# nverchev/PointCloudCounterfactual

Hardware: AMD Instinct MI355X
Metric: clouds/sec Chamfer+EMD fwd+bwd, N=2048 B=32 (higher is better)
Workload: dtype f32; 1 GPU; BASELINE configs[1]+[2]: N=2048 B=32 per GPU, nn_distance (Chamfer, mean) fwd+bwd + match_cost (approxmatch+matchcost) fwd+bwd through the autograd surface; inputs = "recon" clouds (reference permuted + N(0, 0.02^2): a trained autoencoder, SURVEY 8(d)); the 8(d) stress set (both clouds i.i.d. U[0,1]^3) is value_stress (--full); emd_mode=implicit, batch_per_gpu=32, n_points=2048, global_batch=32, parallelism=batch-sharded x1, no data-path collective, launcher=single process

## Files before the change

### pointcloudcounterfactual_amd/backend.py

```python

from __future__ import annotations

import torch

from pointcloudcounterfactual_amd import _lib
from pointcloudcounterfactual_amd._lib import call, ptr

_L = _lib.lib
F32, I32 = torch.float32, torch.int32


def _sizes(set_d: torch.Tensor, set_q: torch.Tensor) -> tuple[int, int, int]:
    return set_d.size(0), set_d.size(1), set_q.size(1)


def ApproxMatch(set_d: torch.Tensor, set_q: torch.Tensor) -> list[torch.Tensor]:
    b, n, m = _sizes(set_d, set_q)
    dev = set_d.device
    match = torch.empty((b, m, n), dtype=torch.float32, device=dev)
    temp = torch.empty((b, (n + m) * 2), dtype=torch.float32, device=dev)
    call(_L.pcc_approxmatch, 'ApproxMatch', dev, b, n, m, ptr(set_d, 'set_d', F32, dev), ptr(set_q, 'set_q', F32, dev),
         ptr(match, 'match', F32, dev), ptr(temp, 'temp', F32, dev))
    return [match, temp]


def ApproxMatchCost(set_d: torch.Tensor, set_q: torch.Tensor) -> list[torch.Tensor]:
    b, n, m = _sizes(set_d, set_q)
    dev = set_d.device
    match = torch.empty((b, m, n), dtype=torch.float32, device=dev)
    temp = torch.empty((b, (n + m) * 2), dtype=torch.float32, device=dev)
    cost = torch.empty((b,), dtype=torch.float32, device=dev)
    call(_L.pcc_approxmatch_cost, 'ApproxMatchCost', dev, b, n, m, ptr(set_d, 'set_d', F32, dev),
         ptr(set_q, 'set_q', F32, dev), ptr(match, 'match', F32, dev), ptr(temp, 'temp', F32, dev),
         ptr(cost, 'cost', F32, dev))
    return [match, temp, cost]


def MatchCostImplicit(set_d: torch.Tensor, set_q: torch.Tensor, with_grad: bool) -> list[torch.Tensor]:
    b, n, m = _sizes(set_d, set_q)
    dev = set_d.device
    cost = torch.empty((b,), dtype=torch.float32, device=dev)
    out = [cost]
    g1 = g2 = None
    if with_grad:
        g1 = torch.empty((b, n, 3), dtype=torch.float32, device=dev)
        g2 = torch.empty((b, m, 3), dtype=torch.float32, device=dev)
        out += [g1, g2]
    call(_L.pcc_match_cost, 'MatchCostImplicit', dev, b, n, m, ptr(set_d, 'set_d', F32, dev),
         ptr(set_q, 'set_q', F32, dev), None, ptr(cost, 'cost', F32, dev), ptr(g1, 'grad1', F32, dev),
         ptr(g2, 'grad2', F32, dev))
    return out


def MatchCost(set_d: torch.Tensor, set_q: torch.Tensor, match: torch.Tensor) -> torch.Tensor:
    b, n, m = _sizes(set_d, set_q)
    dev = set_d.device
    out = torch.empty((b,), dtype=torch.float32, device=dev)
    if match.numel() != b * n * m:
        raise RuntimeError(f'match has {match.numel()} elements, expected {b}x{m}x{n}')
    call(_L.pcc_matchcost, 'MatchCost', dev, b, n, m, ptr(set_d, 'set_d', F32, dev), ptr(set_q, 'set_q', F32, dev),
         ptr(match, 'match', F32, dev), ptr(out, 'cost', F32, dev))
    return out


def MatchCostGrad(set_d: torch.Tensor, set_q: torch.Tensor, match: torch.Tensor) -> list[torch.Tensor]:
    b, n, m = _sizes(set_d, set_q)
    dev = set_d.device
    grad1 = torch.empty((b, n, 3), dtype=torch.float32, device=dev)
    grad2 = torch.empty((b, m, 3), dtype=torch.float32, device=dev)
    if match.numel() != b * n * m:
        raise RuntimeError(f'match has {match.numel()} elements, expected {b}x{m}x{n}')
    call(_L.pcc_matchcostgrad, 'MatchCostGrad', dev, b, n, m, ptr(set_d, 'set_d', F32, dev),
         ptr(set_q, 'set_q', F32, dev), ptr(match, 'match', F32, dev), ptr(grad1, 'grad1', F32, dev),
         ptr(grad2, 'grad2', F32, dev))
    return [grad1, grad2]


def MatchCostGradScaled(set_d: torch.Tensor, set_q: torch.Tensor, match: torch.Tensor,
                        grad_cost: torch.Tensor) -> list[torch.Tensor]:
    b, n, m = _sizes(set_d, set_q)
    dev = set_d.device
    grad1 = torch.empty((b, n, 3), dtype=torch.float32, device=dev)
    grad2 = torch.empty((b, m, 3), dtype=torch.float32, device=dev)
    if match.numel() != b * n * m or grad_cost.numel() != b:
        raise RuntimeError('MatchCostGradScaled: match / grad_cost shapes do not match the clouds')
    call(_L.pcc_matchcostgrad_scaled, 'MatchCostGradScaled', dev, b, n, m, ptr(set_d, 'set_d', F32, dev),
         ptr(set_q, 'set_q', F32, dev), ptr(match, 'match', F32, dev), ptr(grad_cost, 'grad_cost', F32, dev),
         ptr(grad1, 'grad1', F32, dev), ptr(grad2, 'grad2', F32, dev))
    return [grad1, grad2]


def NNDistance(set_d: torch.Tensor, set_q: torch.Tensor) -> list[torch.Tensor]:
    b, n, m = _sizes(set_d, set_q)
    dev = set_d.device
    dist1 = torch.empty((b, n), dtype=torch.float32, device=dev)
    idx1 = torch.empty((b, n), dtype=torch.int32, device=dev)
    dist2 = torch.empty((b, m), dtype=torch.float32, device=dev)
    idx2 = torch.empty((b, m), dtype=torch.int32, device=dev)
    call(_L.pcc_nndistance, 'NNDistance', dev, b, n, ptr(set_d, 'set_d', F32, dev), m, ptr(set_q, 'set_q', F32, dev),
         ptr(dist1, 'dist1', F32, dev), ptr(idx1, 'idx1', I32, dev), ptr(dist2, 'dist2', F32, dev),
         ptr(idx2, 'idx2', I32, dev))
    return [dist1, idx1, dist2, idx2]


def ChamferLoss(set_d: torch.Tensor, set_q: torch.Tensor, mean: bool) -> list[torch.Tensor]:
    b, n, m = _sizes(set_d, set_q)
    dev = set_d.device
    loss = torch.empty((b,), dtype=torch.float32, device=dev)
    dist1 = torch.empty((b, n), dtype=torch.float32, device=dev)
    idx1 = torch.empty((b, n), dtype=torch.int32, device=dev)
    dist2 = torch.empty((b, m), dtype=torch.float32, device=dev)
    idx2 = torch.empty((b, m), dtype=torch.int32, device=dev)
    call(_L.pcc_chamfer_loss, 'ChamferLoss', dev, b, n, ptr(set_d, 'set_d', F32, dev), m, ptr(set_q, 'set_q', F32, dev),
         int(mean), ptr(loss, 'loss', F32, dev), ptr(dist1, 'dist1', F32, dev), ptr(idx1, 'idx1', I32, dev),
         ptr(dist2, 'dist2', F32, dev), ptr(idx2, 'idx2', I32, dev))
    return [loss, dist1, idx1, dist2, idx2]


def ChamferLossGrad(set_d: torch.Tensor, set_q: torch.Tensor, idx1: torch.Tensor, idx2: torch.Tensor,
                    grad_loss: torch.Tensor, mean: bool) -> list[torch.Tensor]:
    b, n, m = _sizes(set_d, set_q)
    dev = set_d.device
    grad1 = torch.empty((b, n, 3), dtype=torch.float32, device=dev)
    grad2 = torch.empty((b, m, 3), dtype=torch.float32, device=dev)
    if idx1.numel() != b * n or idx2.numel() != b * m or grad_loss.numel() != b:
        raise RuntimeError('ChamferLossGrad: idx / grad_loss shapes do not match the clouds')
    grad_loss, stride = _batch_stride(grad_loss, b)
    call(_L.pcc_chamfer_loss_grad, 'ChamferLossGrad', dev, b, n, ptr(set_d, 'set_d', F32, dev), m,
         ptr(set_q, 'set_q', F32, dev), ptr(idx1, 'idx1', I32, dev), ptr(idx2, 'idx2', I32, dev),
         ptr(grad_loss, 'grad_loss', F32, dev), stride, int(mean), ptr(grad1, 'grad1', F32, dev),
         ptr(grad2, 'grad2', F32, dev))
    return [grad1, grad2]


def ChamferEMD(set_d: torch.Tensor, set_q: torch.Tensor, mean: bool, with_grad: bool,
               return_dist: bool = False) -> list[torch.Tensor]:
    b, n, m = _sizes(set_d, set_q)
    dev = set_d.device
    loss = torch.empty((b,), dtype=torch.float32, device=dev)
    idx1 = torch.empty((b, n), dtype=torch.int32, device=dev)
    idx2 = torch.empty((b, m), dtype=torch.int32, device=dev)
    cost = torch.empty((b,), dtype=torch.float32, device=dev)
    out = [loss, idx1, idx2, cost]
    g1 = g2 = None
    if with_grad:
        g1 = torch.empty((b, n, 3), dtype=torch.float32, device=dev)
        g2 = torch.empty((b, m, 3), dtype=torch.float32, device=dev)
        out += [g1, g2]
    d1 = torch.empty((b, n), dtype=torch.float32, device=dev)
    d2 = torch.empty((b, m), dtype=torch.float32, device=dev)
    call(_L.pcc_chamfer_emd, 'ChamferEMD', dev, b, n, ptr(set_d, 'set_d', F32, dev), m, ptr(set_q, 'set_q', F32, dev),
         int(mean), ptr(loss, 'loss', F32, dev), ptr(d1, 'dist1', F32, dev), ptr(idx1, 'idx1', I32, dev),
         ptr(d2, 'dist2', F32, dev), ptr(idx2, 'idx2', I32, dev), ptr(cost, 'cost', F32, dev),
         ptr(g1, 'emd_grad1', F32, dev), ptr(g2, 'emd_grad2', F32, dev))
    if return_dist:
        out += [d1, d2]
    return out


def _batch_stride(g: torch.Tensor, b: int) -> tuple[torch.Tensor, int]:
    stride = g.stride(0) if g.dim() == 1 and b > 1 else 1
    if stride == 0:
        return g[:1], 0
    if stride != 1:
        return g.contiguous(), 1
    return g, 1


def ChamferEMDGrad(set_d: torch.Tensor, set_q: torch.Tensor, idx1: torch.Tensor, idx2: torch.Tensor,
                   grad_chamfer: torch.Tensor, mean: bool, emd_grad1: torch.Tensor, emd_grad2: torch.Tensor,
                   grad_emd: torch.Tensor) -> list[torch.Tensor]:
    b, n, m = _sizes(set_d, set_q)
    dev = set_d.device
    grad1 = torch.empty((b, n, 3), dtype=torch.float32, device=dev)
    grad2 = torch.empty((b, m, 3), dtype=torch.float32, device=dev)
    if (idx1.numel() != b * n or idx2.numel() != b * m or grad_chamfer.numel() != b or grad_emd.numel() != b
            or emd_grad1.numel() != b * n * 3 or emd_grad2.numel() != b * m * 3):
        raise RuntimeError('ChamferEMDGrad: shapes do not match the clouds')
    grad_chamfer, sc = _batch_stride(grad_chamfer, b)
    grad_emd, se = _batch_stride(grad_emd, b)
    call(_L.pcc_chamfer_emd_grad, 'ChamferEMDGrad', dev, b, n, ptr(set_d, 'set_d', F32, dev), m,
         ptr(set_q, 'set_q', F32, dev), ptr(idx1, 'idx1', I32, dev), ptr(idx2, 'idx2', I32, dev),
         ptr(grad_chamfer, 'grad_chamfer', F32, dev), sc, int(mean), ptr(emd_grad1, 'emd_grad1', F32, dev),
         ptr(emd_grad2, 'emd_grad2', F32, dev), ptr(grad_emd, 'grad_emd', F32, dev), se, ptr(grad1, 'grad1', F32, dev),
         ptr(grad2, 'grad2', F32, dev))
    return [grad1, grad2]


def NNDistanceGrad(set_d: torch.Tensor, set_q: torch.Tensor, idx1: torch.Tensor, idx2: torch.Tensor,
                   grad_dist1: torch.Tensor, grad_dist2: torch.Tensor) -> list[torch.Tensor]:
    b, n, m = _sizes(set_d, set_q)
    dev = set_d.device
    grad1 = torch.empty((b, n, 3), dtype=torch.float32, device=dev)
    grad2 = torch.empty((b, m, 3), dtype=torch.float32, device=dev)
    if idx1.numel() != b * n or grad_dist1.numel() != b * n or idx2.numel() != b * m or grad_dist2.numel() != b * m:
        raise RuntimeError('NNDistanceGrad: idx/grad_dist shapes do not match the clouds')
    call(_L.pcc_nndistancegrad, 'NNDistanceGrad', dev, b, n, ptr(set_d, 'set_d', F32, dev), m,
         ptr(set_q, 'set_q', F32, dev), ptr(grad_dist1, 'grad_dist1', F32, dev), ptr(idx1, 'idx1', I32, dev),
         ptr(grad_dist2, 'grad_dist2', F32, dev), ptr(idx2, 'idx2', I32, dev), ptr(grad1, 'grad1', F32, dev),
         ptr(grad2, 'grad2', F32, dev))
    return [grad1, grad2]
```

### pointcloudcounterfactual_amd/csrc/am_pair.hip

```cpp
#include "approxmatch.hpp"
#include "wave_ops.hpp"

#include <algorithm>

namespace {

using pcc::sq3;

constexpr int kPairRB = 8;
constexpr int kPairPad = 65;

struct PairArgs {
    int n, m, n4, m4;
    const float *soa1, *soa2;
    const float *lv;
    LevelConsts lc;
    float cut2[kLevels];
    float *cost_part;
    float *part1;
    float *part2;
    int col_blocks, row_tiles, bc;
};

template <int Q, bool GRAD>
__global__ __launch_bounds__(256) void am_pair_kernel(PairArgs a) {
    __shared__ float4 lds_l[kPairRT][3];
    __shared__ int lds_mask[kPairRT];
    __shared__ float stash[GRAD ? 4 * kPairRB * 3 * kPairPad : 4];
    __shared__ float lds_red[4];
    const int tid = threadIdx.x, lane = tid & 63;
    const int w = __builtin_amdgcn_readfirstlane(tid >> 6);
    const int cbn = a.col_blocks, rtn = a.row_tiles;
    const int item = (int)blockIdx.x / a.bc, smp = (int)blockIdx.x - item * a.bc;
    const int shift_k = item / cbn, cblk = item - shift_k * cbn;
    const int base_r = (int)(((long long)(2 * cblk + 1) * rtn) / (2 * cbn));
    const int shift = ((shift_k + 1) >> 1) * ((shift_k & 1) ? 1 : -1);
    const int rtile = ((base_r + shift) % rtn + rtn) % rtn;
    const int l0 = rtile * kPairRT;
    const int kb = cblk * 64 * Q;
    const int k0 = kb + lane * Q;
    const size_t nm4 = (size_t)a.n4 + a.m4;
    const float *lvb = a.lv + (size_t)smp * kLevels * nm4;
    const float *s1 = a.soa1 + (size_t)smp * 3 * a.n4;
    const float *s2 = a.soa2 + (size_t)smp * 3 * a.m4;
    const int lcnt = min(kPairRT, a.m - l0);

    float rowx = 0.f, rowy = 0.f, rowz = 0.f, rowr[kLevels];
#pragma unroll
    for (int i = 0; i < kLevels; i++) rowr[i] = 0.f;
    if (tid < lcnt) {
        const int l = l0 + tid;
        rowx = s2[l];
        rowy = s2[a.m4 + l];
        rowz = s2[2 * a.m4 + l];
#pragma unroll
        for (int i = 0; i < kLevels; i++) rowr[i] = lvb[(size_t)i * nm4 + a.n4 + l];
    }
    float x1[Q], y1[Q], z1[Q], rl[kLevels][Q];
    float blo[3] = {__builtin_inff(), __builtin_inff(), __builtin_inff()};
    float bhi[3] = {-__builtin_inff(), -__builtin_inff(), -__builtin_inff()};
#pragma unroll
    for (int q = 0; q < Q; q++) {
        const bool real = k0 + q < a.n;
        const int k = real ? k0 + q : a.n - 1;
        x1[q] = s1[k];
        y1[q] = s1[a.n4 + k];
        z1[q] = s1[2 * a.n4 + k];
#pragma unroll
        for (int i = 0; i < kLevels; i++) rl[i][q] = real ? lvb[(size_t)i * nm4 + k] : 0.f;
        blo[0] = fminf(blo[0], x1[q]); bhi[0] = fmaxf(bhi[0], x1[q]);
        blo[1] = fminf(blo[1], y1[q]); bhi[1] = fmaxf(bhi[1], y1[q]);
        blo[2] = fminf(blo[2], z1[q]); bhi[2] = fmaxf(bhi[2], z1[q]);
    }
#pragma unroll
    for (int c = 0; c < 3; c++) {
#pragma unroll
        for (int off = 1; off < 64; off <<= 1) {
            blo[c] = fminf(blo[c], __shfl_xor(blo[c], off, 64));
            bhi[c] = fmaxf(bhi[c], __shfl_xor(bhi[c], off, 64));
        }
    }
    if (tid < lcnt) {
        const float bx = fmaxf(fmaxf(blo[0] - rowx, rowx - bhi[0]), 0.f);
        const float by = fmaxf(fmaxf(blo[1] - rowy, rowy - bhi[1]), 0.f);
        const float bz = fmaxf(fmaxf(blo[2] - rowz, rowz - bhi[2]), 0.f);
        const float bd2 = bx * bx + by * by + bz * bz;
        int mask = 0;
#pragma unroll
        for (int i = 0; i < kLevels; i++) mask |= (rowr[i] != 0.f && !(bd2 > a.cut2[i])) ? (1 << i) : 0;
        lds_l[tid][0] = make_float4(rowx, rowy, rowz, rowr[0]);
        lds_l[tid][1] = make_float4(rowr[1], rowr[2], rowr[3], rowr[4]);
        lds_l[tid][2] = make_float4(rowr[5], rowr[6], rowr[7], rowr[8]);
        lds_mask[tid] = mask;
    }
    float g1[Q][3];
#pragma unroll
    for (int q = 0; q < Q; q++) g1[q][0] = g1[q][1] = g1[q][2] = 0.f;
    float csum = 0.f;
    float *my_stash = stash + (GRAD ? w * kPairRB * 3 * kPairPad : 0);
    __syncthreads();

    for (int base = 0; base < lcnt; base += 4 * kPairRB) {
#pragma unroll 1
        for (int s = 0; s < kPairRB; s++) {
            const int li = base + 4 * s + w;
            float rx = 0.f, ry = 0.f, rz = 0.f;
            const int mask = li < lcnt ? __builtin_amdgcn_readfirstlane(lds_mask[li]) : 0;
            if (mask) {
                const float4 A = lds_l[li][0], B = lds_l[li][1], Cc = lds_l[li][2];
                const float rr[kLevels] = {A.w, B.x, B.y, B.z, B.w, Cc.x, Cc.y, Cc.z, Cc.w};
                float ex[Q], ey[Q], ez[Q], d[Q], acc[Q];
#pragma unroll
                for (int q = 0; q < Q; q++) {
                    ex[q] = A.x - x1[q];
                    ey[q] = A.y - y1[q];
                    ez[q] = A.z - z1[q];
                    d[q] = sq3(ex[q], ey[q], ez[q]);
                    acc[q] = 0.f;
                }
#pragma unroll
                for (int i = 0; i < kLevels; i++) {
                    if (mask & (1 << i)) {
#pragma unroll
                        for (int q = 0; q < Q; q++)
                            acc[q] = __builtin_fmaf(fast_exp2(a.lc.c[i] * d[q]) * rl[i][q], rr[i], acc[q]);
                    }
                }
#pragma unroll
                for (int q = 0; q < Q; q++) {
                    if (GRAD) {
                        float dm;
                        asm("v_max_f32 %0, %1, %2" : "=v"(dm) : "v"(d[q]), "v"(1e-20f));
                        const float f = acc[q] * __builtin_amdgcn_rsqf(dm);
                        csum = __builtin_fmaf(f, d[q], csum);
                        g1[q][0] = __builtin_fmaf(-ex[q], f, g1[q][0]);
                        g1[q][1] = __builtin_fmaf(-ey[q], f, g1[q][1]);
                        g1[q][2] = __builtin_fmaf(-ez[q], f, g1[q][2]);
                        rx = __builtin_fmaf(ex[q], f, rx);
                        ry = __builtin_fmaf(ey[q], f, ry);
                        rz = __builtin_fmaf(ez[q], f, rz);
                    } else {
                        csum = __builtin_fmaf(acc[q], __builtin_amdgcn_sqrtf(d[q]), csum);
                    }
                }
            }
            if (GRAD) {
                my_stash[(s * 3 + 0) * kPairPad + lane] = rx;
                my_stash[(s * 3 + 1) * kPairPad + lane] = ry;
                my_stash[(s * 3 + 2) * kPairPad + lane] = rz;
            }
        }
        if (GRAD) {
            const int v = lane % 24, h = lane / 24;
            float t = 0.f;
            __builtin_amdgcn_wave_barrier();
            if (lane < 48) {
                const float *src = my_stash + v * kPairPad + h * 32;
#pragma unroll 8
                for (int i = 0; i < 32; i++) t += src[i];
            }
            __builtin_amdgcn_wave_barrier();
            const float hi = __shfl(t, lane + 24, 64);
            const int sl = v / 3, c = v - sl * 3;
            const int li = base + 4 * sl + w;
            if (lane < 24 && li < lcnt)
                a.part2[(((size_t)smp * cbn + cblk) * a.m4 + (l0 + li)) * 3 + c] = t + hi;
        }
    }
    csum = pcc::wave_sum_down(csum);
    if (lane == 0) lds_red[w] = csum;
    __syncthreads();
    if (tid == 0)
        a.cost_part[(size_t)smp * cbn * rtn + rtile * cbn + cblk] =
            ((lds_red[0] + lds_red[1]) + lds_red[2]) + lds_red[3];
    if (GRAD) {
        static_assert(Q * 3 * 64 <= 4 * kPairRB * 3 * kPairPad, "column merge reuses the stash");
        for (int src = 1; src < 4; src++) {
            __syncthreads();
            if (w == src) {
#pragma unroll
                for (int q = 0; q < Q; q++)
#pragma unroll
                    for (int c = 0; c < 3; c++) stash[(q * 3 + c) * 64 + lane] = g1[q][c];
            }
            __syncthreads();
            if (w == 0) {
#pragma unroll
                for (int q = 0; q < Q; q++)
#pragma unroll
                    for (int c = 0; c < 3; c++) g1[q][c] += stash[(q * 3 + c) * 64 + lane];
            }
        }
        if (w == 0) {
            float *dst = a.part1 + (((size_t)smp * rtn + rtile) * a.n4) * 3;
#pragma unroll
            for (int q = 0; q < Q; q++) {
                if (k0 + q < a.n) {
#pragma unroll
                    for (int c = 0; c < 3; c++) dst[(size_t)(k0 + q) * 3 + c] = g1[q][c];
                }
            }
        }
    }
}

struct FinishArgs {
    int parts[3], npts[2], pitch[2];
    const float *part[3];
    const int *perm[2];
    const float *scale;
    float *out[3];
    const float *ch_d1, *ch_d2;
    float *ch_loss;
    int ch_n, ch_m, ch_mean;
    const int *flags;
};
__global__ __launch_bounds__(256) void pair_finish_kernel(FinishArgs f) {
    __shared__ float red[256];
    const int which = blockIdx.z, smp = blockIdx.y, tid = threadIdx.x;
    if (which == 3) {
        if (blockIdx.x) return;
        __shared__ float red2[256];
        float s1 = 0.f, s2 = 0.f;
        auto strided_sum = [&](const float *d, int cnt) -> float {
            float acc = 0.f;
            for (int i0 = tid; i0 < cnt; i0 += 8 * 256) {
                float v[8];
#pragma unroll
                for (int u = 0; u < 8; u++) v[u] = d[min(i0 + u * 256, cnt - 1)];
#pragma unroll
                for (int u = 0; u < 8; u++)
                    if (i0 + u * 256 < cnt) acc += v[u];
            }
            return acc;
        };
        s1 = strided_sum(f.ch_d1 + (size_t)smp * f.ch_n, f.ch_n);
        s2 = strided_sum(f.ch_d2 + (size_t)smp * f.ch_m, f.ch_m);
        red[tid] = s1;
        red2[tid] = s2;
        __syncthreads();
        for (int off = 128; off > 0; off >>= 1) {
            if (tid < off) {
                red[tid] += red[tid + off];
                red2[tid] += red2[tid + off];
            }
            __syncthreads();
        }
        if (tid == 0) f.ch_loss[smp] = f.ch_mean ? red2[0] / (float)f.ch_m + red[0] / (float)f.ch_n : red[0] + red2[0];
        return;
    }
    const bool poisoned = f.flags && (f.flags[(size_t)smp * kLiveRow + kInfSlot] | f.flags[(size_t)smp * kLiveRow + kInfSlot + 1] |
                                      f.flags[(size_t)smp * kLiveRow + kErrSlot]);
    if (which == 2) {
        if (blockIdx.x) return;
        const int parts = f.parts[2];
        float s = 0.f;
        for (int i = tid; i < parts; i += 256) s += f.part[2][(size_t)smp * parts + i];
        red[tid] = s;
        __syncthreads();
        for (int off = 128; off > 0; off >>= 1) {
            if (tid < off) red[tid] += red[tid + off];
            __syncthreads();
        }
        if (tid == 0) f.out[2][smp] = poisoned ? __builtin_nanf("") : red[0];
        return;
    }
    if (!f.out[which]) return;
    const int npts = f.npts[which], pitch = f.pitch[which], parts = f.parts[which];
    const int i = blockIdx.x * 256 + tid;
    if (i >= npts * 3) return;
    const int s = i / 3, c = i - s * 3;
    const float *p = f.part[which] + (size_t)smp * parts * pitch * 3 + i;
    const int pt = f.perm[which][(size_t)smp * npts + s];
    const size_t stride = (size_t)pitch * 3;
    float acc = p[0];
    int t = 1;
    for (; t + 8 <= parts; t += 8) {
        float v[8];
#pragma unroll
        for (int u = 0; u < 8; u++) v[u] = p[(size_t)(t + u) * stride];
#pragma unroll
        for (int u = 0; u < 8; u++) acc += v[u];
    }
    {
        float v[7];
#pragma unroll
        for (int u = 0; u < 7; u++) v[u] = p[(size_t)min(t + u, parts - 1) * stride];
#pragma unroll
        for (int u = 0; u < 7; u++)
            if (t + u < parts) acc += v[u];
    }
    f.out[which][((size_t)smp * npts + pt) * 3 + c] = poisoned ? __builtin_nanf("") : f.scale ? acc * f.scale[smp] : acc;
}

template <int Q>
int launch_pair(const PairArgs &pa, dim3 grid, bool grad, hipStream_t st) {
    pcc::ProfScope prof(grad ? "am_pair_kernel<grad>" : "am_pair_kernel<cost>", st);
    if (grad) hipLaunchKernelGGL((am_pair_kernel<Q, true>), grid, dim3(256), 0, st, pa);
    else hipLaunchKernelGGL((am_pair_kernel<Q, false>), grid, dim3(256), 0, st, pa);
    return pcc::check_launch("match_cost(pair)");
}

}

namespace pcc {

int launch_pair_finish(const AmDims &L, const WsView &v, int s0, int bc, int col_blocks, int row_tiles, const float *grad_cost,
                       float *cost, float *grad1, float *grad2, const ChamferOut *chamfer, hipStream_t lst) {
    const size_t o = (size_t)s0;
    const int n = L.n, m = L.m;
    const bool grad = grad1 && grad2;
    const LevelConsts lc = make_levels();
    PairArgs pa{};
    pa.n = n; pa.m = m; pa.n4 = L.n4; pa.m4 = L.m4;
    pa.soa1 = v.soa1; pa.soa2 = v.soa2; pa.lv = v.lv;
    pa.lc = lc;
    for (int i = 0; i < kLevels; i++) pa.cut2[i] = zero_cut2(lc, i);
    pa.cost_part = v.pair_cost;
    pa.part1 = grad ? v.part1 : nullptr;
    pa.part2 = grad ? v.part2 : nullptr;
    pa.col_blocks = col_blocks; pa.row_tiles = row_tiles; pa.bc = bc;
    if ((long long)col_blocks * row_tiles * bc > 0x7fffffffLL) return pcc::invalid("match_cost: grid too large");
    const dim3 grid((unsigned)(col_blocks * row_tiles * bc));
    if (int rc = launch_pair<kPairQ>(pa, grid, grad, lst)) return rc;
    FinishArgs f{};
    f.parts[0] = row_tiles; f.parts[1] = col_blocks; f.parts[2] = col_blocks * row_tiles;
    f.npts[0] = n; f.npts[1] = m; f.pitch[0] = L.n4; f.pitch[1] = L.m4;
    f.part[0] = pa.part1; f.part[1] = pa.part2; f.part[2] = pa.cost_part;
    f.perm[0] = v.perm1; f.perm[1] = v.perm2;
    f.scale = grad_cost ? grad_cost + o : nullptr;
    f.out[0] = grad ? grad1 + o * n * 3 : nullptr;
    f.out[1] = grad ? grad2 + o * m * 3 : nullptr;
    f.out[2] = cost + o;
    f.flags = v.live_cnt;
    if (chamfer) {
        f.ch_d1 = chamfer->dist1 + o * n; f.ch_d2 = chamfer->dist2 + o * m; f.ch_loss = chamfer->loss + o;
        f.ch_n = n; f.ch_m = m; f.ch_mean = chamfer->mean;
    }
    {
        pcc::ProfScope prof("pair_finish_kernel", lst);
        const int blocks = grad ? pcc::ceil_div(std::max(n, m) * 3, 256) : 1;
        hipLaunchKernelGGL(pair_finish_kernel, dim3(blocks, bc, chamfer ? 4 : 3), dim3(256), 0, lst, f);
    }
    return pcc::check_launch("match_cost(reduce)");
}
}
```

### pointcloudcounterfactual_amd/csrc/approxmatch.hip

```cpp
#include "approxmatch.hpp"
#include "pcc_test_hooks.h"
#include "wave_ops.hpp"

#include <algorithm>
#include <functional>
#include <mutex>
#include <type_traits>

namespace {

using pcc::sq3;
using pcc::WsView;

enum Phase { PH_A = 0, PH_B = 1, PH_CA = 2, PH_C = 3 };

__device__ __forceinline__ float pass_a_ratio(float remL, float sum) { return remL / (1e-9f + sum); }
struct PassB {
    float ratio, remain;
};
__device__ __forceinline__ PassB pass_b(float remR, float sum) {
    const float sumr = sum * remR;
    const float consumption = __builtin_fminf(remR / (sumr + 1e-9f), 1.0f);
    return {consumption * remR, __builtin_fmaxf(0.0f, remR - sumr)};
}
__device__ __forceinline__ float pass_c_left(float remL, float ratioL, float sum) { return __builtin_fmaxf(0.0f, remL - ratioL * sum); }

struct PhaseArgs {
    int n_own, n_cand, tiles, batch;
    int own_n4, cand_n4, own_nb, cand_nb;
    const float *own_soa, *cand_soa;
    const float *cand_box;
    const float *own_box16;
    const float *w0, *w1;
    long long w0_stride, w1_stride;
    float w0c;
    float c0, c1;
    float cut2;
    float cut2_fine;
    int first;
    int level;
    float multiL, multiR;
    float *remain;
    float *remain_out;
    long long remain_stride;
    const float *ratio_in;
    float *ratio_out;
    long long ratio_stride;
    float *clist;
    int *clist_cnt;
    int cl_n4;
    const unsigned *mask_in;
    unsigned *mask_out;
    int mask_words;
    const int *live_in;
    int *live_out;
};

enum Var { V_PLAIN = 0, V_CULL = 1, V_COWN = 3, V_CLIST = 4 };

struct Sched {
    int n, m, n4, m4, nb1, nb2;
    const float *soa1, *soa2, *box1, *box2;
    float *rem, *lv;
    float multiL, multiR;
    float *clist;
    int *clist_cnt;
    int *live_cnt;
    unsigned *live_mask;
    int skip;
    LevelConsts lc;
};

inline int sched_phases() { return 2 * kLevels + 1; }

inline PhaseArgs build_phase(const Sched &sc, int p, int *mode_out, int *var_out) {
    const long long nm4 = (long long)sc.n4 + sc.m4;
    const long long rs = (long long)sc.n4 + 2LL * sc.m4;
    PhaseArgs a{};
    a.multiL = sc.multiL;
    a.multiR = sc.multiR;
    const bool set1_owns = (p == 0) || (p % 2 == 0);
    if (set1_owns) {
        a.n_own = sc.n; a.n_cand = sc.m; a.own_n4 = sc.n4; a.cand_n4 = sc.m4; a.own_nb = sc.nb1; a.cand_nb = sc.nb2;
        a.own_soa = sc.soa1; a.cand_soa = sc.soa2; a.cand_box = sc.box2;
        a.own_box16 = sc.box1;
    } else {
        a.n_own = sc.m; a.n_cand = sc.n; a.own_n4 = sc.m4; a.cand_n4 = sc.n4; a.own_nb = sc.nb2; a.cand_nb = sc.nb1;
        a.own_soa = sc.soa2; a.cand_soa = sc.soa1; a.cand_box = sc.box1;
        a.own_box16 = sc.box2;
    }
    int mode, var;
    if (p == 0) {
        mode = PH_A;
        var = sc.skip ? V_CULL : V_PLAIN;
        a.level = 0;
        a.w0 = nullptr; a.w0c = sc.multiR; a.c0 = sc.lc.c[0]; a.first = 1;
        a.cut2 = zero_cut2(sc.lc, 0);
        a.ratio_out = sc.lv; a.ratio_stride = kLevels * nm4;
    } else {
        const int i = (p - 1) / 2;
        float *ratioL = sc.lv + (size_t)i * nm4, *ratioR = ratioL + sc.n4;
        a.level = i;
        a.first = (i == 0);
        a.c0 = sc.lc.c[i];
        if (p % 2 == 1) {
            mode = PH_B;
            var = !sc.skip ? V_PLAIN : i <= 2 ? V_CULL : V_COWN;
            a.w0 = ratioL; a.w0_stride = kLevels * nm4;
            a.cut2 = zero_cut2(sc.lc, i);
            a.remain = sc.rem + sc.n4 + (i & 1) * sc.m4;
            a.remain_out = sc.rem + sc.n4 + ((i + 1) & 1) * sc.m4;
            a.remain_stride = rs;
            a.ratio_out = ratioR; a.ratio_stride = kLevels * nm4;
            if (var == V_COWN) { a.clist = sc.clist; a.clist_cnt = sc.clist_cnt; a.cl_n4 = sc.m4; }
            if (sc.live_mask) {
                const int words = mask_words(sc.m4);
                a.mask_words = words;
                if (i + 1 < kLevels && (var == V_COWN || i == 2)) a.mask_out = sc.live_mask + (size_t)(i + 1) * words;
                if (var == V_COWN) {
                    a.mask_in = sc.live_mask + (size_t)i * words;
                    a.remain = a.remain_out = sc.rem + sc.n4 + sc.m4;
                }
            }
            if (sc.live_cnt) {
                a.live_in = (var == V_COWN && i >= 1) ? sc.live_cnt + i : nullptr;
                a.live_out = i + 1 < kLevels ? sc.live_cnt + i + 1 : nullptr;
            }
        } else {
            mode = i + 1 < kLevels ? PH_CA : PH_C;
            var = !sc.skip ? V_PLAIN : i <= 2 ? V_CULL : V_CLIST;
            if (var == V_CLIST) { a.clist = sc.clist; a.clist_cnt = sc.clist_cnt; a.cl_n4 = sc.m4; }
            a.w0 = ratioR; a.w0_stride = kLevels * nm4;
            a.w1 = sc.rem + sc.n4 + ((i + 1) & 1) * sc.m4; a.w1_stride = rs;
            a.remain = sc.rem; a.remain_stride = rs;
            a.ratio_in = ratioL; a.ratio_stride = kLevels * nm4;
            const int lc_i = i + 1 < kLevels ? i + 1 : i;
            a.cut2 = zero_cut2(sc.lc, lc_i);
            a.cut2_fine = zero_cut2(sc.lc, i);
            if (i + 1 < kLevels) {
                a.c1 = sc.lc.c[i + 1];
                a.ratio_out = sc.lv + (size_t)(i + 1) * nm4;
            }
        }
    }
    *mode_out = mode;
    *var_out = var;
    return a;
}

template <int NW, int R, int S, int CH>
struct PhaseLds {
    static constexpr int kC = (3 + NW) * CH;
    static constexpr int kRed = NW * S * 64 * R;
    static constexpr int kOwn = 64 * R;
    static constexpr int kWave = S;
    static constexpr int floats = kC + kRed + kOwn + kWave + 4;
};

template <int MODE, int R, int S, int CH, int VAR, int G = 1>
__device__ __forceinline__ void am_phase_body(const PhaseArgs &a, int smp, int tile, float *smem) {
    constexpr int T = 64 * S;
    constexpr int TQ = 64 * R / G;
    constexpr int PQ = 64 * R;
    static_assert(G == 1 || (VAR == V_COWN && R == 1), "lane-split owners: owner-compacted launches only");
    constexpr int NW = (MODE == PH_CA) ? 2 : 1;
    constexpr bool W0_CONST = (MODE == PH_A);
    constexpr bool COWN = VAR == V_COWN, CLIST = VAR == V_CLIST;
    static_assert(VAR == V_PLAIN || COWN || CLIST, "the box-culled passes run on am_fine_kernel");
    static_assert(!(CLIST && W0_CONST), "pass A of the first level has constant weights");
    static_assert(TQ <= T, "one epilogue owner per thread");
    using L = PhaseLds<NW, R, S, CH>;
    float *lds_c = smem;
    float *red = smem + L::kC;
    int *own_idx = reinterpret_cast<int *>(red + L::kRed);
    int *wave_cnt = own_idx + L::kOwn;

    const int tid = threadIdx.x;
    const int lane = tid & 63;
    const int w = __builtin_amdgcn_readfirstlane(tid >> 6);
    const int sub = G > 1 ? lane / TQ : 0;
    const float *O = a.own_soa + (size_t)smp * 3 * a.own_n4;
    const float *C = a.cand_soa + (size_t)smp * 3 * a.cand_n4;
    const float *W0 = W0_CONST ? nullptr : a.w0 + (size_t)smp * a.w0_stride;
    const float *W1 = (NW == 2) ? a.w1 + (size_t)smp * a.w1_stride : nullptr;

    if (!COWN && tile * TQ >= a.n_own) return;
    static_assert(CH / 4 <= T, "one float4 group per thread and chunk");
    float4 st_x, st_y, st_z, st_0, st_1;
    auto stage_load = [&](const float *Cc, const float *W0c, const float *W1c, int pitch, int q0, int ngroups) {
        const int i = min(tid, max(ngroups - 1, 0));
        st_x = reinterpret_cast<const float4 *>(Cc + q0)[i];
        st_y = reinterpret_cast<const float4 *>(Cc + (size_t)pitch + q0)[i];
        st_z = reinterpret_cast<const float4 *>(Cc + (size_t)2 * pitch + q0)[i];
        st_0 = make_float4(a.w0c, a.w0c, a.w0c, a.w0c);
        st_1 = st_0;
        if (!W0_CONST) st_0 = *reinterpret_cast<const float4 *>(W0c + q0 + 4 * i);
        if (NW == 2) st_1 = *reinterpret_cast<const float4 *>(W1c + q0 + 4 * i);
    };
    if (COWN) stage_load(C, W0, W1, a.cand_n4, 0, (min(CH, a.n_cand) + 3) / 4);
    int n_valid = min(TQ, a.n_own - tile * TQ);
    if (COWN) {
        const int lo = tile * TQ, hi = lo + TQ;
        const unsigned *mk = a.mask_in + (size_t)smp * kLevels * a.mask_words;
        unsigned *mnext = (tile == 0 && a.mask_out) ? a.mask_out + (size_t)smp * kLevels * a.mask_words : nullptr;
        const int wpt = (a.mask_words + T - 1) / T;
        unsigned word = 0;
        int mine = 0;
        if (wpt == 1) {
            word = mk[min(tid, a.mask_words - 1)];
            word &= -(unsigned)(tid < a.mask_words);
            if (mnext && tid < a.mask_words) atomicAnd(&mnext[tid], word);
            mine = __popc(word);
        } else {
            for (int j = tid * wpt; j < min(tid * wpt + wpt, a.mask_words); j++) {
                const unsigned wj = mk[j];
                if (mnext) atomicAnd(&mnext[j], wj);
                mine += __popc(wj);
            }
        }
        int incl = mine;
#pragma unroll
        for (int off = 1; off < 64; off <<= 1) {
            const int v = __shfl_up(incl, off, 64);
            incl += lane >= off ? v : 0;
        }
        if (lane == 63) wave_cnt[w] = incl;
        __syncthreads();
        int before = 0, total = 0;
#pragma unroll
        for (int i = 0; i < S; i++) {
            const int c = __builtin_amdgcn_readfirstlane(wave_cnt[i]);
            before += i < w ? c : 0;
            total += c;
        }
        int pos = before + incl - mine - lo;
        auto deal = [&](unsigned bits, int first_owner) {
            while (bits) {
                const int bit = __builtin_ctz(bits);
                bits &= bits - 1;
                if ((unsigned)pos < (unsigned)TQ) own_idx[pos] = first_owner + bit;
                pos++;
            }
        };
        if (wpt == 1) {
            deal(word, tid * 32);
        } else {
            for (int j = tid * wpt; j < min(tid * wpt + wpt, a.mask_words); j++) deal(mk[j], j * 32);
        }
        if (a.clist_cnt && tile == 0 && tid == 0) a.clist_cnt[smp] = total;
        n_valid = min(TQ, total - lo);
        if (n_valid <= 0) return;
        (void)hi;
        __syncthreads();
    }
    int own_e = -1;
    if (tid < TQ && tid < n_valid) own_e = COWN ? own_idx[tid] : tile * TQ + tid;

    float ox[R], oy[R], oz[R], s0[R], s1[R];
    float t0x = 0.f, t1x = 0.f;
#pragma unroll
    for (int r = 0; r < R; r++) {
        const int e = G > 1 ? (lane & (TQ - 1)) : r * 64 + lane;
        int o = COWN ? own_idx[e < n_valid ? e : 0] : tile * TQ + e;
        o = o < a.n_own ? o : a.n_own - 1;
        ox[r] = O[o];
        oy[r] = O[a.own_n4 + o];
        oz[r] = O[2 * a.own_n4 + o];
        s0[r] = 0.f;
        s1[r] = 0.f;
    }
    float pre_rem = 0.f, pre_ratio = 0.f;
    {
        const int oe = max(own_e, 0);
        if (MODE != PH_A && !a.first) pre_rem = a.remain[(size_t)smp * a.remain_stride + oe];
        if (MODE == PH_CA || MODE == PH_C) pre_ratio = a.ratio_in[(size_t)smp * a.ratio_stride + oe];
    }
    const float4 *X4 = reinterpret_cast<const float4 *>(lds_c);
    const float4 *Y4 = X4 + CH / 4;
    const float4 *Z4 = Y4 + CH / 4;
    const float4 *A4 = Z4 + CH / 4;
    const float4 *B4 = A4 + CH / 4;
    const float c0 = a.c0, c1 = a.c1;

    const int n_cand = CLIST ? __builtin_amdgcn_readfirstlane(a.clist_cnt[smp]) : a.n_cand;
    if (CLIST) {
        C = a.clist + (size_t)smp * 5 * a.cl_n4;
        W0 = C + (size_t)3 * a.cl_n4;
        W1 = C + (size_t)4 * a.cl_n4;
    }
    const int cand_pitch = CLIST ? a.cl_n4 : a.cand_n4;
    for (int q0 = 0; q0 < n_cand; q0 += CH) {
        const int cnt = min(CH, n_cand - q0);
        int ngroups = (cnt + 3) / 4;
        if (q0) __syncthreads();
        {
            float4 *dst4 = reinterpret_cast<float4 *>(lds_c);
            if (!(COWN && q0 == 0)) stage_load(C, W0, W1, cand_pitch, q0, ngroups);
            const int i = tid;
            if (i < ngroups) {
                float4 vx = st_x, vy = st_y, vz = st_z, v0 = st_0, v1 = st_1;
                if (CLIST && i * 4 + 3 >= cnt) {
                    vx.y = i * 4 + 1 < cnt ? vx.y : 0.f; vx.z = i * 4 + 2 < cnt ? vx.z : 0.f; vx.w = 0.f;
                    vy.y = i * 4 + 1 < cnt ? vy.y : 0.f; vy.z = i * 4 + 2 < cnt ? vy.z : 0.f; vy.w = 0.f;
                    vz.y = i * 4 + 1 < cnt ? vz.y : 0.f; vz.z = i * 4 + 2 < cnt ? vz.z : 0.f; vz.w = 0.f;
                }
                if ((W0_CONST || CLIST) && i * 4 + 3 >= cnt) {
                    v0.x = i * 4 + 0 < cnt ? v0.x : 0.f;
                    v0.y = i * 4 + 1 < cnt ? v0.y : 0.f;
                    v0.z = i * 4 + 2 < cnt ? v0.z : 0.f;
                    v0.w = 0.f;
                    if (NW == 2) {
                        v1.x = i * 4 + 0 < cnt ? v1.x : 0.f;
                        v1.y = i * 4 + 1 < cnt ? v1.y : 0.f;
                        v1.z = i * 4 + 2 < cnt ? v1.z : 0.f;
                        v1.w = 0.f;
                    }
                }
                dst4[i] = vx;
                dst4[CH / 4 + i] = vy;
                dst4[2 * (CH / 4) + i] = vz;
                dst4[3 * (CH / 4) + i] = v0;
                if (NW == 2) dst4[4 * (CH / 4) + i] = v1;
            }
        }
        const int nblk = (ngroups + 3) / 4;
        __syncthreads();
        for (int blk = w; blk < nblk; blk += S) {
            const int g_end = min(blk * 4 + 4, ngroups);
            for (int g = blk * 4 + sub; g < g_end; g += G) {
                const float4 x = X4[g], y = Y4[g], z = Z4[g], wa = A4[g];
                float4 wb;
                if (NW == 2) wb = B4[g];
#pragma unroll
                for (int r = 0; r < R; r++) {
                    const float d0 = sq3(x.x - ox[r], y.x - oy[r], z.x - oz[r]);
                    const float d1 = sq3(x.y - ox[r], y.y - oy[r], z.y - oz[r]);
                    const float d2 = sq3(x.z - ox[r], y.z - oy[r], z.z - oz[r]);
                    const float d3 = sq3(x.w - ox[r], y.w - oy[r], z.w - oz[r]);
                    if (R == 1) {
                        s0[r] = __builtin_fmaf(fast_exp2(c0 * d0), wa.x, s0[r]);
                        t0x = __builtin_fmaf(fast_exp2(c0 * d1), wa.y, t0x);
                        s0[r] = __builtin_fmaf(fast_exp2(c0 * d2), wa.z, s0[r]);
                        t0x = __builtin_fmaf(fast_exp2(c0 * d3), wa.w, t0x);
                        if (NW == 2) {
                            s1[r] = __builtin_fmaf(fast_exp2(c1 * d0), wb.x, s1[r]);
                            t1x = __builtin_fmaf(fast_exp2(c1 * d1), wb.y, t1x);
                            s1[r] = __builtin_fmaf(fast_exp2(c1 * d2), wb.z, s1[r]);
                            t1x = __builtin_fmaf(fast_exp2(c1 * d3), wb.w, t1x);
                        }
                    } else {
                        s0[r] = __builtin_fmaf(fast_exp2(c0 * d0), wa.x, s0[r]);
                        s0[r] = __builtin_fmaf(fast_exp2(c0 * d1), wa.y, s0[r]);
                        s0[r] = __builtin_fmaf(fast_exp2(c0 * d2), wa.z, s0[r]);
                        s0[r] = __builtin_fmaf(fast_exp2(c0 * d3), wa.w, s0[r]);
                        if (NW == 2) {
                            s1[r] = __builtin_fmaf(fast_exp2(c1 * d0), wb.x, s1[r]);
                            s1[r] = __builtin_fmaf(fast_exp2(c1 * d1), wb.y, s1[r]);
                            s1[r] = __builtin_fmaf(fast_exp2(c1 * d2), wb.z, s1[r]);
                            s1[r] = __builtin_fmaf(fast_exp2(c1 * d3), wb.w, s1[r]);
                        }
                    }
                }
            }
        }
    }
    if (R == 1) {
        s0[0] += t0x;
        s1[0] += t1x;
    }
    if (G > 1) {
        s0[0] += __shfl_xor(s0[0], TQ, 64);
        if (G == 4) s0[0] += __shfl_xor(s0[0], 2 * TQ, 64);
    }
#pragma unroll
    for (int r = 0; r < R; r++) {
        red[(0 * S + w) * PQ + r * 64 + lane] = s0[r];
        if (NW == 2) red[(1 * S + w) * PQ + r * 64 + lane] = s1[r];
    }
    __syncthreads();
    if (own_e < 0) return;
    {
        const int e = tid;
        const int o = own_e;
        float t0 = red[e], t1 = 0.f;
        if (NW == 2) t1 = red[(1 * S) * PQ + e];
#pragma unroll
        for (int s = 1; s < S; s++) {
            t0 += red[(0 * S + s) * PQ + e];
            if (NW == 2) t1 += red[(1 * S + s) * PQ + e];
        }
        if (MODE == PH_A) {
            a.ratio_out[(size_t)smp * a.ratio_stride + o] = pass_a_ratio(a.multiL, t0);
        } else if (MODE == PH_B) {
            const PassB pb = pass_b(a.first ? a.multiR : pre_rem, t0);
            const float ratio_new = pb.ratio, remain_new = pb.remain;
            a.ratio_out[(size_t)smp * a.ratio_stride + o] = ratio_new;
            a.remain_out[(size_t)smp * a.remain_stride + o] = remain_new;
            if (a.live_out) {
                const unsigned long long alive = __ballot(remain_new != 0.f);
                if (lane == 0) atomicAdd(&a.live_out[(size_t)smp * kLiveRow], (int)__popcll(alive));
            }
            if (COWN && a.mask_out && remain_new == 0.f)
                atomicAnd(&a.mask_out[(size_t)smp * kLevels * a.mask_words + (o >> 5)], ~(1u << (o & 31)));
            if (COWN && a.clist) {
                float cx = ox[0], cy = oy[0], cz = oz[0];
#pragma unroll
                for (int r = 1; r < R; r++) {
                    cx = w == r ? ox[r] : cx;
                    cy = w == r ? oy[r] : cy;
                    cz = w == r ? oz[r] : cz;
                }
                float *cl = a.clist + (size_t)smp * 5 * a.cl_n4 + tile * TQ + e;
                cl[0] = cx;
                cl[(size_t)a.cl_n4] = cy;
                cl[(size_t)2 * a.cl_n4] = cz;
                cl[(size_t)3 * a.cl_n4] = ratio_new;
                cl[(size_t)4 * a.cl_n4] = remain_new;
            }
        } else {
            const float left = pass_c_left(a.first ? a.multiL : pre_rem, pre_ratio, t0);
            a.remain[(size_t)smp * a.remain_stride + o] = left;
            if (MODE == PH_CA) a.ratio_out[(size_t)smp * a.ratio_stride + o] = pass_a_ratio(left, t1);
        }
    }
}

template <int MODE, int R, int S, int CH, int VAR, int G = 1>
__global__ __launch_bounds__(64 * S) void am_phase_kernel(PhaseArgs a) {
    __shared__ __attribute__((aligned(16))) float smem[PhaseLds<(MODE == PH_CA ? 2 : 1), R, S, CH>::floats];
    constexpr bool COWN = VAR == V_COWN;
    int smp, tile;
    const int bid = (int)blockIdx.x, nwg = (int)gridDim.x;
    if (COWN) {
        if (a.batch % 8 == 0) {
            const int per = a.batch / 8, i = bid / 8;
            smp = (bid % 8) + 8 * (i % per);
            tile = i / per;
        } else {
            smp = bid % a.batch;
            tile = bid / a.batch;
        }
        if (a.live_in && tile > 0 && tile * (64 * R / G) >= a.live_in[(size_t)smp * kLiveRow]) return;
    } else {
        const int lid = pcc::xcd_contiguous(bid, nwg);
        smp = lid / a.tiles;
        tile = lid - smp * a.tiles;
    }
    am_phase_body<MODE, R, S, CH, VAR, G>(a, smp, tile, smem);
}

constexpr int kFineS = 8;
constexpr int kFineOG = 16;
constexpr int kFineGroups = 64 / kFineOG;
constexpr int kFineQ = 4;

struct FineOwners {
    float x[kFineQ], y[kFineQ], z[kFineQ];
};
struct FineRows {
    const float *x, *y, *z, *w0, *w1;
};

__device__ __forceinline__ void fine_group_box(const float *own_box, int own_nb, int smp, int g16, float4 &lo, float4 &hi) {
    lo = make_float4(__builtin_inff(), __builtin_inff(), __builtin_inff(), 0.f);
    hi = make_float4(-__builtin_inff(), -__builtin_inff(), -__builtin_inff(), 0.f);
    if (g16 < own_nb) {
        const float4 *ob = reinterpret_cast<const float4 *>(own_box + ((size_t)smp * own_nb + g16) * 8);
        lo = ob[0];
        hi = ob[1];
    }
}

__device__ __forceinline__ float fine_box_d2(const float4 &glo, const float4 &ghi, const float *cand_box) {
    const float4 *cb = reinterpret_cast<const float4 *>(cand_box);
    const float4 lo = cb[0], hi = cb[1];
    const float dx = fmaxf(fmaxf(glo.x - hi.x, lo.x - ghi.x), 0.f);
    const float dy = fmaxf(fmaxf(glo.y - hi.y, lo.y - ghi.y), 0.f);
    const float dz = fmaxf(fmaxf(glo.z - hi.z, lo.z - ghi.z), 0.f);
    return dx * dx + dy * dy + dz * dz;
}

template <int NBLK>
__device__ __forceinline__ void fine_block_list(bool keep, bool outer_only, int tid, int tg, int tb, int w, int lane,
                                                int *wave_cnt, unsigned char (*items)[NBLK], unsigned char *need) {
    if (tid < NBLK) need[tid] = 0;
    const unsigned long long bal = __ballot(keep);
    if (lane == 0) wave_cnt[w] = __popcll(bal);
    __syncthreads();
    const int before = (w & 1) ? wave_cnt[w - 1] : 0;
    if (keep) {
        items[tg][before + __popcll(bal & ((1ull << lane) - 1ull))] = (unsigned char)(tb | (outer_only ? 128 : 0));
        need[tb] = 1;
    }
    __syncthreads();
}

template <int NW>
__device__ __forceinline__ void fine_walk(const FineRows &rows, const unsigned char *list, int nitems, int cs, int cl, float c0,
                                          float c1, const FineOwners &own, float (&s0)[kFineQ], float (&s1)[kFineQ]) {
    for (int it = cs; it < nitems; it += 2) {
        const int item = __builtin_amdgcn_readfirstlane((int)list[it]);
        const int ci = (item & 127) * kBox + cl;
        const float x = rows.x[ci], y = rows.y[ci], z = rows.z[ci];
        if (NW == 2 && (item & 128)) {
            const float wb = rows.w1[ci];
#pragma unroll
            for (int j = 0; j < kFineQ; j++) s1[j] = __builtin_fmaf(fast_exp2(c1 * sq3(x - own.x[j], y - own.y[j], z - own.z[j])), wb, s1[j]);
            continue;
        }
        const float wa = rows.w0[ci];
        float wb = 0.f;
        if (NW == 2) wb = rows.w1[ci];
#pragma unroll
        for (int j = 0; j < kFineQ; j++) {
            const float d = sq3(x - own.x[j], y - own.y[j], z - own.z[j]);
            s0[j] = __builtin_fmaf(fast_exp2(c0 * d), wa, s0[j]);
            if (NW == 2) s1[j] = __builtin_fmaf(fast_exp2(c1 * d), wb, s1[j]);
        }
    }
}

template <int NW>
__device__ __forceinline__ void fine_reduce(float (&s0)[kFineQ], float (&s1)[kFineQ], float (*red)[2][64], int cs, int cl, int og, int quad) {
    const auto add = [](float a, float b) { return a + b; };
#pragma unroll
    for (int j = 0; j < kFineQ; j++) {
        s0[j] = pcc::row_reduce16(s0[j], add);
        if (NW == 2) s1[j] = pcc::row_reduce16(s1[j], add);
    }
    if (cl == 0) {
#pragma unroll
        for (int j = 0; j < kFineQ; j++) {
            red[0][cs][og * kFineOG + quad * kFineQ + j] = s0[j];
            if (NW == 2) red[1][cs][og * kFineOG + quad * kFineQ + j] = s1[j];
        }
    }
}

template <int MODE, int CH>
__global__ __launch_bounds__(64 * kFineS, MODE == PH_CA ? 4 : 8) void am_fine_kernel(PhaseArgs a) {
    constexpr int T = 64 * kFineS;
    constexpr int NW = (MODE == PH_CA) ? 2 : 1;
    constexpr bool W0_CONST = (MODE == PH_A);
    constexpr int NBLK = CH / kBox;
    static_assert(kFineGroups * NBLK == T, "one (owner group, candidate block) box test per thread");
    static_assert(kFineOG == kBox && kFineOG * kFineQ == 64, "a wave = 16 candidates x 4 owner quads");
    __shared__ __attribute__((aligned(16))) float lds_c[(3 + NW) * CH];
    __shared__ float red[NW][2][64];
    __shared__ unsigned char items[kFineGroups][NBLK];
    __shared__ unsigned char need[NBLK];
    __shared__ int wave_cnt[kFineS];

    const int lid = pcc::xcd_contiguous((int)blockIdx.x, (int)gridDim.x);
    const int smp = lid / a.tiles;
    const int tile = lid - smp * a.tiles;
    const int tid = threadIdx.x, lane = tid & 63;
    const int w = __builtin_amdgcn_readfirstlane(tid >> 6);
    const int og = w & (kFineGroups - 1);
    const int cs = w / kFineGroups;
    const int cl = lane & (kBox - 1);
    const int quad = lane / kBox;
    const float *O = a.own_soa + (size_t)smp * 3 * a.own_n4;
    const float *C = a.cand_soa + (size_t)smp * 3 * a.cand_n4;
    const float *W0 = W0_CONST ? nullptr : a.w0 + (size_t)smp * a.w0_stride;
    const float *W1 = (NW == 2) ? a.w1 + (size_t)smp * a.w1_stride : nullptr;

    FineOwners own;
    float s0[kFineQ], s1[kFineQ];
#pragma unroll
    for (int j = 0; j < kFineQ; j++) {
        int o = tile * 64 + og * kFineOG + quad * kFineQ + j;
        o = o < a.n_own ? o : a.n_own - 1;
        own.x[j] = O[o];
        own.y[j] = O[a.own_n4 + o];
        own.z[j] = O[2 * a.own_n4 + o];
        s0[j] = 0.f;
        s1[j] = 0.f;
    }
    const int own_e = (tid < 64 && tile * 64 + tid < a.n_own) ? tile * 64 + tid : -1;
    float pre_rem = 0.f, pre_ratio = 0.f;
    {
        const int oe = max(own_e, 0);
        if (MODE != PH_A && !a.first) pre_rem = a.remain[(size_t)smp * a.remain_stride + oe];
        if (MODE == PH_CA || MODE == PH_C) pre_ratio = a.ratio_in[(size_t)smp * a.ratio_stride + oe];
    }
    const int tg = tid / NBLK, tb = tid - tg * NBLK;
    float4 glo, ghi;
    fine_group_box(a.own_box16, a.own_nb, smp, tile * kFineGroups + tg, glo, ghi);
    const float c0 = a.c0, c1 = a.c1, cut2 = a.cut2;
    const FineRows rows = {lds_c, lds_c + CH, lds_c + 2 * CH, lds_c + 3 * CH, lds_c + 4 * CH};

    for (int q0 = 0; q0 < a.n_cand; q0 += CH) {
        const int cnt = min(CH, a.n_cand - q0);
        const int ngroups = (cnt + 3) / 4;
        const int nblk = (ngroups + 3) / 4;
        if (q0) __syncthreads();
        bool keep = false, outer_only = false;
        if (tb < nblk) {
            const float bd2 = fine_box_d2(glo, ghi, a.cand_box + ((size_t)smp * a.cand_nb + q0 / kBox + tb) * 8);
            keep = !(bd2 > cut2);
            outer_only = NW == 2 && bd2 > a.cut2_fine;
        }
        fine_block_list<NBLK>(keep, outer_only, tid, tg, tb, w, lane, wave_cnt, items, need);
        {
            float4 *dst4 = reinterpret_cast<float4 *>(lds_c);
            const float4 *sx = reinterpret_cast<const float4 *>(C + q0);
            const float4 *sy = reinterpret_cast<const float4 *>(C + (size_t)a.cand_n4 + q0);
            const float4 *sz = reinterpret_cast<const float4 *>(C + (size_t)2 * a.cand_n4 + q0);
            static_assert(CH / 4 <= T, "one float4 group per thread and chunk");
            const int i = tid;
            if (i < nblk * 4 && need[i >> 2]) {
                float4 vx = make_float4(0.f, 0.f, 0.f, 0.f), vy = vx, vz = vx, v0 = vx, v1 = vx;
                if (i < ngroups) {
                    vx = sx[i]; vy = sy[i]; vz = sz[i];
                    v0 = W0_CONST ? make_float4(a.w0c, a.w0c, a.w0c, a.w0c) : *reinterpret_cast<const float4 *>(W0 + q0 + 4 * i);
                    if (NW == 2) v1 = *reinterpret_cast<const float4 *>(W1 + q0 + 4 * i);
                    if (W0_CONST && i * 4 + 3 >= cnt) {
                        v0.x = i * 4 + 0 < cnt ? v0.x : 0.f;
                        v0.y = i * 4 + 1 < cnt ? v0.y : 0.f;
                        v0.z = i * 4 + 2 < cnt ? v0.z : 0.f;
                        v0.w = 0.f;
                    }
                }
                dst4[i] = vx;
                dst4[CH / 4 + i] = vy;
                dst4[2 * (CH / 4) + i] = vz;
                dst4[3 * (CH / 4) + i] = v0;
                if (NW == 2) dst4[4 * (CH / 4) + i] = v1;
            }
        }
        __syncthreads();
        fine_walk<NW>(rows, items[og], wave_cnt[2 * og] + wave_cnt[2 * og + 1], cs, cl, c0, c1, own, s0, s1);
    }
    fine_reduce<NW>(s0, s1, red, cs, cl, og, quad);
    __syncthreads();
    if (own_e < 0) return;
    const float sum0 = red[0][0][tid] + red[0][1][tid];
    const float sum1 = NW == 2 ? red[NW - 1][0][tid] + red[NW - 1][1][tid] : 0.f;
    if (MODE == PH_A) {
        a.ratio_out[(size_t)smp * a.ratio_stride + own_e] = pass_a_ratio(a.multiL, sum0);
    } else if (MODE == PH_B) {
        const PassB pb = pass_b(a.first ? a.multiR : pre_rem, sum0);
        a.ratio_out[(size_t)smp * a.ratio_stride + own_e] = pb.ratio;
        a.remain_out[(size_t)smp * a.remain_stride + own_e] = pb.remain;
        if (a.live_out) {
            const unsigned long long alive = __ballot(pb.remain != 0.f);
            if (lane == 0) atomicAdd(&a.live_out[(size_t)smp * kLiveRow], (int)__popcll(alive));
            if (a.mask_out && lane == 0) {
                unsigned *mo = a.mask_out + (size_t)smp * kLevels * a.mask_words;
                if (2 * tile < a.mask_words) mo[2 * tile] = (unsigned)alive;
                if (2 * tile + 1 < a.mask_words) mo[2 * tile + 1] = (unsigned)(alive >> 32);
            }
        }
    } else {
        const float left = pass_c_left(a.first ? a.multiL : pre_rem, pre_ratio, sum0);
        a.remain[(size_t)smp * a.remain_stride + own_e] = left;
        if (MODE == PH_CA) a.ratio_out[(size_t)smp * a.ratio_stride + own_e] = pass_a_ratio(left, sum1);
    }
}

constexpr int kFpPasses = 7;
constexpr int kFpCH = 2048;

struct FinePersistArgs {
    int n, m, n4, m4, nb1, nb2, tiles;
    const float *soa1, *soa2, *box1, *box2;
    float *rem, *lv;
    float multiL, multiR;
    float c[4], cut2[4];
    int *live_cnt;
    unsigned *live_mask;
    int mask_words;
    unsigned *host_err;
    int inject;
};

__global__ __launch_bounds__(64 * kFineS) void am_fine_persist_kernel(FinePersistArgs a) {
    constexpr int T = 64 * kFineS, CH = kFpCH, NBLK = CH / kBox;
    static_assert(kFineGroups * NBLK == T, "one (owner group, candidate block) box test per thread and direction");
    __shared__ __attribute__((aligned(16))) float lds_p[2][3 * CH];
    __shared__ __attribute__((aligned(16))) float lds_w[2][CH];
    __shared__ float red[2][2][64];
    __shared__ unsigned char items[kFineGroups][NBLK];
    __shared__ unsigned char need[NBLK];
    __shared__ int wave_cnt[kFineS];

    const int lid = pcc::xcd_contiguous((int)blockIdx.x, (int)gridDim.x);
    const int smp = lid / a.tiles;
    const int tile = lid - smp * a.tiles;
    const int tid = threadIdx.x, lane = tid & 63;
    const int w = __builtin_amdgcn_readfirstlane(tid >> 6);
    const int og = w & (kFineGroups - 1), cs = w / kFineGroups;
    const int cl = lane & (kBox - 1), quad = lane / kBox;
    const long long nm4 = (long long)a.n4 + a.m4, rs = (long long)a.n4 + 2LL * a.m4;
    const float *S1 = a.soa1 + (size_t)smp * 3 * a.n4;
    const float *S2 = a.soa2 + (size_t)smp * 3 * a.m4;
    float *LV = a.lv + (size_t)smp * kLevels * nm4;
    float *REM = a.rem + (size_t)smp * rs;
    int *row = a.live_cnt + (size_t)smp * kLiveRow;
    unsigned *bar = reinterpret_cast<unsigned *>(row + kBarSlot);
    unsigned *err = reinterpret_cast<unsigned *>(row + kErrSlot);

    for (int s = 0; s < 2; s++) {
        const float *S = s ? S2 : S1;
        const int p4 = s ? a.m4 : a.n4, ngroups = p4 / 4, nblk = (ngroups + 3) / 4;
        float4 *dst4 = reinterpret_cast<float4 *>(lds_p[s]);
        const float4 *sx = reinterpret_cast<const float4 *>(S);
        const float4 *sy = reinterpret_cast<const float4 *>(S + p4);
        const float4 *sz = reinterpret_cast<const float4 *>(S + 2 * (size_t)p4);
        for (int i = tid; i < nblk * 4; i += T) {
            float4 vx = make_float4(0.f, 0.f, 0.f, 0.f), vy = vx, vz = vx;
            if (i < ngroups) { vx = sx[i]; vy = sy[i]; vz = sz[i]; }
            dst4[i] = vx;
            dst4[CH / 4 + i] = vy;
            dst4[2 * (CH / 4) + i] = vz;
        }
    }
    FineOwners set1, set2;
#pragma unroll
    for (int j = 0; j < kFineQ; j++) {
        const int o = tile * 64 + og * kFineOG + quad * kFineQ + j;
        const int o1 = min(o, a.n - 1), o2 = min(o, a.m - 1);
        set1.x[j] = S1[o1]; set1.y[j] = S1[a.n4 + o1]; set1.z[j] = S1[2 * a.n4 + o1];
        set2.x[j] = S2[o2]; set2.y[j] = S2[a.m4 + o2]; set2.z[j] = S2[2 * a.m4 + o2];
    }
    const int tg = tid / NBLK, tb = tid - tg * NBLK;
    auto box_d2 = [&](const float *own_box, int own_nb, const float *cand_box, int cand_nb) -> float {
        float4 glo, ghi;
        fine_group_box(own_box, own_nb, smp, tile * kFineGroups + tg, glo, ghi);
        if (tb >= cand_nb) return __builtin_inff();
        return fine_box_d2(glo, ghi, cand_box + ((size_t)smp * cand_nb + tb) * 8);
    };
    const float d2_role0 = box_d2(a.box1, a.nb1, a.box2, a.nb2);
    const float d2_role1 = box_d2(a.box2, a.nb2, a.box1, a.nb1);
    const int own1 = (tid < 64 && tile * 64 + tid < a.n) ? tile * 64 + tid : -1;
    const int own2 = (tid < 64 && tile * 64 + tid < a.m) ? tile * 64 + tid : -1;
    float remL = 0.f, ratL = 0.f, remR = 0.f;
    unsigned arrivals = 0;
    bool ok = true;

    auto pass = [&](auto mode_tag, int i) {
        constexpr int MODE = decltype(mode_tag)::value;
        constexpr int NW = MODE == PH_CA ? 2 : 1;
        constexpr int ROLE = MODE == PH_B ? 1 : 0;
        const int n_cand = ROLE ? a.n : a.m, cand_n4 = ROLE ? a.n4 : a.m4;
        const int nblk = (cand_n4 / 4 + 3) / 4;
        const float c0 = a.c[i], c1 = a.c[MODE == PH_CA ? i + 1 : i];
        const float cut2 = a.cut2[MODE == PH_CA ? i + 1 : i];
        const float *P = lds_p[ROLE ? 0 : 1];
        const float bd2 = ROLE ? d2_role1 : d2_role0;
        const bool keep = tb < nblk && !(bd2 > cut2);
        const bool outer_only = NW == 2 && bd2 > a.cut2[i];
        fine_block_list<NBLK>(keep, outer_only, tid, tg, tb, w, lane, wave_cnt, items, need);
        {
            const float *W0 = MODE == PH_A ? nullptr : MODE == PH_B ? LV + (size_t)i * nm4 : LV + (size_t)i * nm4 + a.n4;
            const float *W1 = MODE == PH_CA ? REM + a.n4 + (size_t)((i + 1) & 1) * a.m4 : nullptr;
            for (int idx = tid; idx < nblk * kBox; idx += T) {
                if (!need[idx >> 4]) continue;
                float v0, v1 = 0.f;
                if (MODE == PH_A) v0 = idx < n_cand ? a.multiR : 0.f;
                else v0 = idx < cand_n4 ? pcc::agent_ld(W0 + idx) : 0.f;
                if (NW == 2) v1 = idx < cand_n4 ? pcc::agent_ld(W1 + idx) : 0.f;
                lds_w[0][idx] = v0;
                if (NW == 2) lds_w[1][idx] = v1;
            }
        }
        __syncthreads();
        float s0[kFineQ], s1[kFineQ];
#pragma unroll
        for (int j = 0; j < kFineQ; j++) s0[j] = s1[j] = 0.f;
        const FineRows rows = {P, P + CH, P + 2 * CH, lds_w[0], lds_w[1]};
        fine_walk<NW>(rows, items[og], wave_cnt[2 * og] + wave_cnt[2 * og + 1], cs, cl, c0, c1, ROLE ? set2 : set1, s0, s1);
        fine_reduce<NW>(s0, s1, red, cs, cl, og, quad);
        __syncthreads();
        const int own_e = ROLE ? own2 : own1;
        if (own_e >= 0) {
            const float sum0 = red[0][0][tid] + red[0][1][tid];
            const float sum1 = NW == 2 ? red[1][0][tid] + red[1][1][tid] : 0.f;
            if (MODE == PH_A) {
                ratL = pass_a_ratio(a.multiL, sum0);
                pcc::agent_st(LV + own_e, ratL);
            } else if (MODE == PH_B) {
                const PassB pb = pass_b(i == 0 ? a.multiR : remR, sum0);
                pcc::agent_st(LV + (size_t)i * nm4 + a.n4 + own_e, pb.ratio);
                pcc::agent_st(REM + a.n4 + (size_t)((i + 1) & 1) * a.m4 + own_e, pb.remain);
                remR = pb.remain;
                if (i == 2) {
                    const unsigned long long alive = __ballot(pb.remain != 0.f);
                    if (lane == 0) {
                        atomicAdd(&row[3], (int)__popcll(alive));
                        unsigned *mo = a.live_mask + ((size_t)smp * kLevels + 3) * a.mask_words;
                        if (2 * tile < a.mask_words) mo[2 * tile] = (unsigned)alive;
                        if (2 * tile + 1 < a.mask_words) mo[2 * tile + 1] = (unsigned)(alive >> 32);
                    }
                }
            } else {
                remL = pass_c_left(i == 0 ? a.multiL : remL, ratL, sum0);
                pcc::agent_st(REM + own_e, remL);
                ratL = pass_a_ratio(remL, sum1);
                pcc::agent_st(LV + (size_t)(i + 1) * nm4 + own_e, ratL);
            }
        }
    };
    auto barrier = [&]() -> bool {
        arrivals += (unsigned)a.tiles;
        return pcc::coresident_barrier<1, (1u << 22)>(bar, arrivals, err, a.host_err, [&] {
            const unsigned seen = pcc::agent_ld(bar);
            return 1u | ((arrivals / (unsigned)a.tiles) << 4) | ((seen & 0xfffu) << 8) | ((unsigned)smp << 20);
        });
    };
    if (a.inject && tile == 0 && tid == 0) pcc::coresident_fail(err, a.host_err, 1u | ((unsigned)smp << 20));
    __syncthreads();
    pass(std::integral_constant<int, PH_A>{}, 0);
    for (int i = 0; i < 3 && ok; i++) {
        ok = barrier();
        if (!ok) break;
        pass(std::integral_constant<int, PH_B>{}, i);
        ok = barrier();
        if (!ok) break;
        pass(std::integral_constant<int, PH_CA>{}, i);
    }
}

__global__ __launch_bounds__(256) void am_unpermute_kernel(int n, int m, int n4, int m4,
                                                            const float *__restrict__ lv_sorted,
                                                            const float *__restrict__ rem_sorted,
                                                            const int *__restrict__ rank1,
                                                            const int *__restrict__ rank2,
                                                            const int *__restrict__ flags,
                                                            float *__restrict__ lv, float *__restrict__ temp) {
    const int smp = blockIdx.y;
    const int i = blockIdx.x * 256 + threadIdx.x;
    if (i >= n + m) return;
    const int s = i < n ? rank1[(size_t)smp * n + i] : n4 + rank2[(size_t)smp * m + (i - n)];
    const size_t nm = (size_t)n + m, nm4 = (size_t)n4 + m4;
    const float *src = lv_sorted + (size_t)smp * kLevels * nm4;
    float *dst = lv + (size_t)smp * kLevels * nm;
    const bool failed = flags[(size_t)smp * kLiveRow + kErrSlot] != 0;
    float last = 0.f;
#pragma unroll
    for (int l = 0; l < kLevels; l++) {
        last = failed ? __builtin_nanf("") : src[(size_t)l * nm4 + s];
        dst[(size_t)l * nm + i] = last;
    }
    float *tb = temp + (size_t)smp * 2 * nm;
    tb[i] = failed ? __builtin_nanf("") : rem_sorted[(size_t)smp * (nm4 + m4) + (i < n ? s : s + m4)];
    tb[nm + i] = last;
}

constexpr int kMatLT = 64;
constexpr int kMatKT = 256;

template <bool COST, bool VEC>
__global__ __launch_bounds__(256) void am_materialise_kernel(int n, int m, const float *__restrict__ xyz1,
                                                              const float *__restrict__ xyz2,
                                                              const float *__restrict__ lv, LevelConsts lc,
                                                              float *__restrict__ match,
                                                              float *__restrict__ cost_part) {
    __shared__ float4 lds_l[kMatLT][3];
    __shared__ float lds_red[4];
    const int tid = threadIdx.x, lane = tid & 63;
    const int w = __builtin_amdgcn_readfirstlane(tid >> 6);
    const int smp = blockIdx.z;
    const int l0 = blockIdx.y * kMatLT;
    const int k0 = blockIdx.x * kMatKT + lane * 4;
    const size_t lvs = (size_t)kLevels * (n + m);
    const float *lvb = lv + (size_t)smp * lvs;
    const float *p1 = xyz1 + (size_t)smp * n * 3;
    const float *p2 = xyz2 + (size_t)smp * m * 3;
    const int lcnt = min(kMatLT, m - l0);

    if (tid < lcnt) {
        const int l = l0 + tid;
        float rr[kLevels];
#pragma unroll
        for (int i = 0; i < kLevels; i++) rr[i] = lvb[(size_t)i * (n + m) + n + l];
        lds_l[tid][0] = make_float4(p2[l * 3 + 0], p2[l * 3 + 1], p2[l * 3 + 2], rr[0]);
        lds_l[tid][1] = make_float4(rr[1], rr[2], rr[3], rr[4]);
        lds_l[tid][2] = make_float4(rr[5], rr[6], rr[7], rr[8]);
    }
    float x1[4], y1[4], z1[4], rl[kLevels][4];
#pragma unroll
    for (int q = 0; q < 4; q++) {
        int k = k0 + q;
        k = k < n ? k : n - 1;
        x1[q] = p1[k * 3 + 0];
        y1[q] = p1[k * 3 + 1];
        z1[q] = p1[k * 3 + 2];
#pragma unroll
        for (int i = 0; i < kLevels; i++) rl[i][q] = lvb[(size_t)i * (n + m) + k];
    }
    __syncthreads();
    float csum = 0.f;
    for (int li = w; li < lcnt; li += 4) {
        const float4 A = lds_l[li][0], B = lds_l[li][1], Cc = lds_l[li][2];
        const float rr[kLevels] = {A.w, B.x, B.y, B.z, B.w, Cc.x, Cc.y, Cc.z, Cc.w};
        int live[kLevels];
#pragma unroll
        for (int i = 0; i < kLevels; i++) live[i] = __builtin_amdgcn_readfirstlane((int)(rr[i] != 0.f));
        float d[4], acc[4];
#pragma unroll
        for (int q = 0; q < 4; q++) {
            d[q] = sq3(A.x - x1[q], A.y - y1[q], A.z - z1[q]);
            acc[q] = 0.f;
        }
#pragma unroll
        for (int i = 0; i < kLevels; i++) {
            if (live[i]) {
#pragma unroll
                for (int q = 0; q < 4; q++) acc[q] += (fast_exp2(lc.c[i] * d[q]) * rl[i][q]) * rr[i];
            }
        }
        float out[4];
#pragma unroll
        for (int q = 0; q < 4; q++) {
            out[q] = acc[q];
            if (COST && k0 + q < n) csum = __builtin_fmaf(acc[q], __builtin_amdgcn_sqrtf(d[q]), csum);
        }
        float *row = match + ((size_t)smp * m + (l0 + li)) * n;
        if (VEC) {
            if (k0 + 3 < n) {
                v4f o4 = {out[0], out[1], out[2], out[3]};
                __builtin_nontemporal_store(o4, reinterpret_cast<v4f *>(row + k0));
            } else {
#pragma unroll
                for (int q = 0; q < 4; q++)
                    if (k0 + q < n) row[k0 + q] = out[q];
            }
        } else {
#pragma unroll
            for (int q = 0; q < 4; q++)
                if (k0 + q < n) row[k0 + q] = out[q];
        }
    }
    if (COST) {
        csum = pcc::wave_sum_down(csum);
        if (lane == 0) lds_red[w] = csum;
        __syncthreads();
        if (tid == 0)
            cost_part[(size_t)smp * gridDim.x * gridDim.y + blockIdx.y * gridDim.x + blockIdx.x] =
                ((lds_red[0] + lds_red[1]) + lds_red[2]) + lds_red[3];
    }
}

constexpr int kPhCH = 2048;
constexpr int kClistCH = 1024;

static bool cull_enabled() {
    return pcc::tuning(PCC_TUNE_AM_NOCULL) == 0;
}

template <int MODE>
const char *phase_name(int level) {
    static const char *const names[4][kLevels] = {
        {"am_phase_kernel<A> L0", "", "", "", "", "", "", "", ""},
        {"am_phase_kernel<B> L0", "am_phase_kernel<B> L1", "am_phase_kernel<B> L2", "am_phase_kernel<B> L3",
         "am_phase_kernel<B> L4", "am_phase_kernel<B> L5", "am_phase_kernel<B> L6", "am_phase_kernel<B> L7",
         "am_phase_kernel<B> L8"},
        {"am_phase_kernel<CA> L0", "am_phase_kernel<CA> L1", "am_phase_kernel<CA> L2", "am_phase_kernel<CA> L3",
         "am_phase_kernel<CA> L4", "am_phase_kernel<CA> L5", "am_phase_kernel<CA> L6", "am_phase_kernel<CA> L7", ""},
        {"", "", "", "", "", "", "", "", "am_phase_kernel<C> L8"}};
    return names[MODE][level];
}

template <int MODE, int R, int S, int G = 1>
int launch_phase_rs(PhaseArgs a, int b, int var, hipStream_t st, const char *what) {
    a.tiles = pcc::ceil_div(a.n_own, 64 * R / G);
    a.batch = b;
    const long long grid = (long long)b * a.tiles;
    if (grid > 0x7fffffffLL) return pcc::invalid("approxmatch: grid too large");
    {
        pcc::ProfScope prof(phase_name<MODE>(a.level), st);
        const dim3 g((unsigned)grid), blk(64 * S);
        if (var == V_CLIST && (MODE == PH_CA || MODE == PH_C))
            hipLaunchKernelGGL((am_phase_kernel<(MODE == PH_CA || MODE == PH_C) ? MODE : PH_C, R, S, kClistCH, V_CLIST>), g, blk, 0, st, a);
        else if (var == V_COWN && MODE == PH_B)
            hipLaunchKernelGGL((am_phase_kernel<PH_B, (G > 1 ? 1 : R), S, kPhCH, V_COWN, G>), g, blk, 0, st, a);
        else hipLaunchKernelGGL((am_phase_kernel<MODE, R, S, kPhCH, V_PLAIN>), g, blk, 0, st, a);
    }
    return pcc::check_launch(what);
}

template <int MODE>
int launch_fine(PhaseArgs a, int b, hipStream_t st, const char *what) {
    a.tiles = pcc::ceil_div(a.n_own, 64);
    a.batch = b;
    const long long grid = (long long)b * a.tiles;
    if (grid > 0x7fffffffLL) return pcc::invalid("approxmatch: grid too large");
    {
        pcc::ProfScope prof(phase_name<MODE>(a.level), st);
        hipLaunchKernelGGL((am_fine_kernel<(MODE == PH_C ? PH_CA : MODE), kPhCH>), dim3((unsigned)grid), dim3(64 * kFineS), 0, st, a);
    }
    return pcc::check_launch(what);
}

template <int MODE>
int launch_phase(const PhaseArgs &a, int b, int var, hipStream_t st, const char *what) {
    if (var == V_CULL) return launch_fine<MODE>(a, b, st, what);
    if (var == V_COWN) {
        if (a.live_in && a.level >= 5) return launch_phase_rs<MODE, 1, 8, 4>(a, b, var, st, what);
        if (a.live_in && a.level >= 4) return launch_phase_rs<MODE, 1, 8, 2>(a, b, var, st, what);
        return launch_phase_rs<MODE, 1, 8>(a, b, var, st, what);
    }
    const long long owners = (long long)b * a.n_own;
    if (var == V_CLIST && owners < 4LL * 65536) return launch_phase_rs<MODE, 1, 8>(a, b, var, st, what);
    if (owners >= 4LL * 65536) return launch_phase_rs<MODE, 4, 8>(a, b, var, st, what);
    if (owners >= 32768) return launch_phase_rs<MODE, 2, 8>(a, b, var, st, what);
    return launch_phase_rs<MODE, 1, 8>(a, b, var, st, what);
}

size_t cost_parts(int n, int m) { return (size_t)pcc::ceil_div(n, kMatKT) * pcc::ceil_div(m, kMatLT); }

struct WsLayout : pcc::AmDims {
    int b;
    int col_blocks, row_tiles;
    bool grad;
    size_t total;
    WsLayout(int b_, int n_, int m_, int col_blocks_ = 0, int row_tiles_ = 0, bool grad_ = false)
        : AmDims(n_, m_), b(b_), col_blocks(col_blocks_), row_tiles(row_tiles_), grad(grad_) {
        WsView unused;
        total = carve(0, 0, unused);
    }
    WsView view(char *base, int s) const {
        WsView v;
        carve(reinterpret_cast<uintptr_t>(base), (size_t)s, v);
        return v;
    }

  private:
    size_t carve(uintptr_t base, size_t s, WsView &v) const {
        size_t o = 0;
        auto sec = [&](auto *&p, size_t per) {
            using T = std::remove_reference_t<decltype(*p)>;
            p = reinterpret_cast<T *>(base + o + s * per * sizeof(T));
            o = (o + (size_t)b * per * sizeof(T) + 15) & ~(size_t)15;
        };
        sec(v.soa1, 3 * (size_t)n4);
        sec(v.soa2, 3 * (size_t)m4);
        sec(v.rank1, n);
        sec(v.rank2, m);
        sec(v.perm1, n);
        sec(v.perm2, m);
        sec(v.box1, (size_t)nb1 * 8);
        sec(v.box2, (size_t)nb2 * 8);
        sec(v.rem, rem_floats());
        sec(v.lv, lv_floats());
        sec(v.lv_orig, kLevels * ((size_t)n + m));
        sec(v.cpart, cost_parts(n, m));
        sec(v.clist, 5 * (size_t)m4);
        sec(v.clist_cnt, 1);
        sec(v.live_cnt, kLiveRow);
        sec(v.live_mask, (size_t)kLevels * mask_words(m4));
        sec(v.aos1, n);
        sec(v.aos2, m);
        sec(v.pair_cost, (size_t)col_blocks * row_tiles);
        sec(v.part1, grad ? (size_t)row_tiles * n4 * 3 : 0);
        sec(v.part2, grad ? (size_t)col_blocks * m4 * 3 : 0);
        return o;
    }
};

constexpr int kMaxLanes = 2;
hipStream_t side_stream() {
    static std::mutex mu;
    static hipStream_t streams[64] = {};
    int dev = 0;
    if (hipGetDevice(&dev) != hipSuccess || dev < 0 || dev >= 64) return nullptr;
    std::lock_guard<std::mutex> lk(mu);
    if (!streams[dev]) {
        int least = 0, greatest = 0;
        if (hipDeviceGetStreamPriorityRange(&least, &greatest) != hipSuccess) {
            (void)hipGetLastError();
            least = greatest = 0;
        }
        if (hipStreamCreateWithPriority(&streams[dev], hipStreamNonBlocking, greatest) != hipSuccess) {
            (void)hipGetLastError();
            if (hipStreamCreateWithFlags(&streams[dev], hipStreamNonBlocking) != hipSuccess) {
                streams[dev] = nullptr;
                (void)hipGetLastError();
            }
        }
    }
    return streams[dev];
}

struct ForkJoin {
    hipStream_t main, side = nullptr;
    ForkJoin(hipStream_t m, bool fork) : main(m) {
        if (!fork) return;
        hipEvent_t ev;
        if (hipEventCreateWithFlags(&ev, hipEventDisableTiming) != hipSuccess) return;
        if (hipEventRecord(ev, main) == hipSuccess) {
            hipStream_t s = side_stream();
            if (s && hipStreamWaitEvent(s, ev, 0) == hipSuccess) side = s;
        }
        (void)hipEventDestroy(ev);
    }
    ~ForkJoin() {
        if (!side) return;
        hipEvent_t ev;
        if (hipEventCreateWithFlags(&ev, hipEventDisableTiming) != hipSuccess) {
            (void)hipStreamSynchronize(side);
            return;
        }
        (void)hipEventRecord(ev, side);
        (void)hipStreamWaitEvent(main, ev, 0);
        (void)hipEventDestroy(ev);
    }
};

static bool resident_enabled() {
    return pcc::tuning(PCC_TUNE_AM_NORESIDENT) == 0;
}
int launch_fine_resident(const Sched &sc, int bc, hipStream_t st) {
    if (!sc.skip || !sc.live_cnt || !sc.live_mask || !resident_enabled()) return -1;
    if (sc.n > kFpCH || sc.m > kFpCH || sc.n < 1 || sc.m < 1) return -1;
    const int tiles = pcc::ceil_div(std::max(sc.n, sc.m), 64);
    FinePersistArgs a{};
    a.n = sc.n; a.m = sc.m; a.n4 = sc.n4; a.m4 = sc.m4; a.nb1 = sc.nb1; a.nb2 = sc.nb2; a.tiles = tiles;
    a.soa1 = sc.soa1; a.soa2 = sc.soa2; a.box1 = sc.box1; a.box2 = sc.box2;
    a.rem = sc.rem; a.lv = sc.lv; a.multiL = sc.multiL; a.multiR = sc.multiR;
    for (int i = 0; i < 4; i++) {
        a.c[i] = sc.lc.c[i];
        a.cut2[i] = zero_cut2(sc.lc, i);
    }
    a.live_cnt = sc.live_cnt;
    a.live_mask = sc.live_mask;
    a.mask_words = mask_words(sc.m4);
    static const int per_cu = [] {
        int r = 0;
        const void *k = reinterpret_cast<const void *>(am_fine_persist_kernel);
        if (hipOccupancyMaxActiveBlocksPerMultiprocessor(&r, k, 64 * kFineS, 0) != hipSuccess) (void)hipGetLastError();
        return r;
    }();
    if (per_cu < 2 || (long long)bc * tiles > pcc::device_cus()) return -1;
    pcc::CoresidentGate gate(pcc::kFineResident, st);
    if (!gate.ok) return -1;
    a.host_err = gate.sticky;
    a.inject = gate.inject;
    {
        pcc::ProfScope prof("am_fine_persist_kernel", st);
        hipLaunchKernelGGL(am_fine_persist_kernel, dim3((unsigned)(bc * tiles)), dim3(64 * kFineS), 0, st, a);
    }
    return pcc::check_launch("approxmatch(resident fine levels)");
}

Sched lane_sched(const WsLayout &L, const WsView &v, const LevelConsts &lc) {
    Sched sc{};
    sc.n = L.n; sc.m = L.m; sc.n4 = L.n4; sc.m4 = L.m4; sc.nb1 = L.nb1; sc.nb2 = L.nb2;
    sc.soa1 = v.soa1; sc.soa2 = v.soa2; sc.box1 = v.box1; sc.box2 = v.box2; sc.rem = v.rem; sc.lv = v.lv;
    if (L.n >= L.m) { sc.multiL = 1; sc.multiR = (float)(L.n / L.m); }
    else { sc.multiL = (float)(L.m / L.n); sc.multiR = 1; }
    sc.skip = cull_enabled() ? 1 : 0;
    sc.lc = lc;
    sc.clist = v.clist; sc.clist_cnt = v.clist_cnt;
    if (sc.skip) { sc.live_cnt = v.live_cnt; sc.live_mask = v.live_mask; }
    return sc;
}

int run_levels(const WsLayout &L, char *base, const float *xyz1, const float *xyz2, const LevelConsts &lc, hipStream_t st,
               const std::function<int(int, int, hipStream_t)> &lane_tail = nullptr,
               const std::function<int(int, int, hipStream_t)> &after_sort = nullptr) {
    if (const unsigned fw = pcc::take_coresident_failure(pcc::kFineResident)) {
        char buf[320];
        std::snprintf(buf, sizeof buf, "approxmatch: an earlier call on this device did not complete (a sample barrier of the resident "
                      "fine-level launch timed out: barrier %u of sample %u saw %u arrivals; the implicit path reported NaN for those "
                      "samples); this call was not started", (fw >> 4) & 0xfu, fw >> 20, (fw >> 8) & 0xfffu);
        return pcc::invalid(buf);
    }
    const bool split_enabled = pcc::tuning(PCC_TUNE_AM_NOSPLIT) == 0;

    struct Lane {
        int s0, bc;
        hipStream_t st;
        WsView v;
        Sched sc;
    };
    Lane lanes[kMaxLanes];
    int nlanes = 1;
    bool fork = false;
    if (split_enabled && L.b >= 8 && (long long)L.b * std::max(L.n, L.m) >= 32768) {
        fork = !pcc::capturing(st);
    }
    ForkJoin fj(st, fork);
    if (fj.side) nlanes = 2;
    for (int l = 0; l < nlanes; l++) {
        Lane &ln = lanes[l];
        ln.s0 = (int)((long long)L.b * l / nlanes);
        ln.bc = (int)((long long)L.b * (l + 1) / nlanes) - ln.s0;
        ln.st = l == 0 ? st : fj.side;
        ln.v = L.view(base, ln.s0);
        ln.sc = lane_sched(L, ln.v, lc);
    }
    int rc = PCC_OK;
    auto enqueue_head = [&](int l) -> int {
        const Lane &ln = lanes[l];
        const size_t s0 = (size_t)ln.s0;
        int r = pcc::sort_clouds(L, ln.v, ln.bc, xyz1 + s0 * L.n * 3, xyz2 + s0 * L.m * 3, (bool)after_sort, ln.st);
        if (!r && after_sort && l % 2 == 0) r = after_sort(ln.s0, ln.bc, ln.st);
        return r;
    };
    auto enqueue_pass = [&](int l, int p) -> int {
        const Lane &ln = lanes[l];
        int mode, var;
        const PhaseArgs a = build_phase(ln.sc, p, &mode, &var);
        switch (mode) {
        case PH_A: return launch_phase<PH_A>(a, ln.bc, var, ln.st, "approxmatch(A)");
        case PH_B: return launch_phase<PH_B>(a, ln.bc, var, ln.st, "approxmatch(B)");
        case PH_CA: return launch_phase<PH_CA>(a, ln.bc, var, ln.st, "approxmatch(CA)");
        default: return launch_phase<PH_C>(a, ln.bc, var, ln.st, "approxmatch(C)");
        }
    };
    int first_pass[kMaxLanes] = {};
    {
        for (int l = 0; l < nlanes && !rc; l++) rc = enqueue_head(l);
        if (rc) return rc;
        {
            pcc::ProfScope seq0("am_phase_sequence", lanes[0].st, true);
            pcc::ProfScope seq1("am_phase_sequence", lanes[nlanes > 1 ? 1 : 0].st, true, nlanes >= 2);
            for (int l = 0; l < nlanes && !rc; l++) {
                const int r = launch_fine_resident(lanes[l].sc, lanes[l].bc, lanes[l].st);
                if (r > 0) rc = r;
                else if (r == 0) first_pass[l] = kFpPasses;
            }
            for (int p = 0; p < sched_phases() && !rc; p++)
                for (int l = 0; l < nlanes && !rc; l++)
                    if (p >= first_pass[l]) rc = enqueue_pass(l, p);
            if (rc) return rc;
        }
        if (after_sort)
            for (int l = 1; l < nlanes; l += 2)
                if (int rc2 = after_sort(lanes[l].s0, lanes[l].bc, lanes[l].st)) return rc2;
        if (lane_tail) {
            for (int l = 0; l < nlanes; l++)
                if (int rc2 = lane_tail(lanes[l].s0, lanes[l].bc, lanes[l].st)) return rc2;
        }
    }
    return PCC_OK;
}

int approxmatch_impl(int b, int n, int m, const float *xyz1, const float *xyz2, float *match, float *temp,
                     void *workspace, size_t workspace_bytes, float *cost_out, hipStream_t st) {
    const WsLayout L(b, n, m);
    if (workspace_bytes < L.total) return pcc::invalid("approxmatch: workspace too small");
    if (!aligned16(workspace)) return pcc::invalid("approxmatch: workspace must be 16-byte aligned");
    char *base = static_cast<char *>(workspace);
    const LevelConsts lc = make_levels();
    int rc = run_levels(L, base, xyz1, xyz2, lc, st);
    if (rc) return rc;
    const WsView v = L.view(base, 0);
    hipLaunchKernelGGL(am_unpermute_kernel, dim3(pcc::ceil_div(n + m, 256), b), dim3(256), 0, st, n, m, L.n4, L.m4, v.lv, v.rem,
                       v.rank1, v.rank2, v.live_cnt, v.lv_orig, temp);
    rc = pcc::check_launch("approxmatch(unpermute)");
    if (rc) return rc;
    const dim3 grid(pcc::ceil_div(n, kMatKT), pcc::ceil_div(m, kMatLT), b);
    const bool vec = (n % 4 == 0) && aligned16(match);
    if (cost_out) {
        {
            pcc::ProfScope prof("am_materialise_kernel<cost>", st);
            if (vec) hipLaunchKernelGGL((am_materialise_kernel<true, true>), grid, dim3(256), 0, st, n, m, xyz1, xyz2, v.lv_orig, lc, match, v.cpart);
            else hipLaunchKernelGGL((am_materialise_kernel<true, false>), grid, dim3(256), 0, st, n, m, xyz1, xyz2, v.lv_orig, lc, match, v.cpart);
        }
        rc = pcc::check_launch("approxmatch(materialise+cost)");
        if (rc) return rc;
        pcc::launch_reduce_rows(b, (int)cost_parts(n, m), v.cpart, cost_out, st);
        return pcc::check_launch("approxmatch(cost reduce)");
    }
    {
        pcc::ProfScope prof("am_materialise_kernel", st);
        if (vec) hipLaunchKernelGGL((am_materialise_kernel<false, true>), grid, dim3(256), 0, st, n, m, xyz1, xyz2, v.lv_orig, lc, match, nullptr);
        else hipLaunchKernelGGL((am_materialise_kernel<false, false>), grid, dim3(256), 0, st, n, m, xyz1, xyz2, v.lv_orig, lc, match, nullptr);
    }
    return pcc::check_launch("approxmatch(materialise)");
}

int match_cost_implicit_impl(int b, int n, int m, const float *xyz1, const float *xyz2, const float *grad_cost,
                             float *cost, float *grad1, float *grad2, hipStream_t st,
                             const pcc::ChamferOut *chamfer = nullptr) {
    const bool grad = grad1 && grad2;
    const int col_blocks = pcc::ceil_div(n, 64 * kPairQ), row_tiles = pcc::ceil_div(m, kPairRT);
    const WsLayout L(b, n, m, col_blocks, row_tiles, grad);
    pcc::WsBlock ws(st);
    if (int rc = ws.alloc(L.total, "workspace allocation failed")) return rc;
    char *base = static_cast<char *>(ws.p);
    const LevelConsts lc = make_levels();
    auto tail = [&](int s0, int bc, hipStream_t lst) -> int {
        return pcc::launch_pair_finish(L, L.view(base, s0), s0, bc, col_blocks, row_tiles, grad_cost, cost, grad1, grad2, chamfer, lst);
    };
    auto nn_after_sort = [&](int s0, int bc, hipStream_t lst) -> int {
        return pcc::launch_nn_sorted(L, L.view(base, s0), s0, bc, chamfer, lst);
    };
    if (chamfer) return run_levels(L, base, xyz1, xyz2, lc, st, tail, nn_after_sort);
    return run_levels(L, base, xyz1, xyz2, lc, st, tail);
}

int approxmatch_entry(int b, int n, int m, const float *xyz1, const float *xyz2, float *match, float *temp, bool with_cost,
                      float *cost, hipStream_t st) {
    pcc::clear_error();
    if (int rc = check_sizes(with_cost ? "approxmatch_cost: bad size" : "approxmatch: bad size", b, n, m)) return rc;
    const char *null_ptr = with_cost ? "approxmatch_cost: null pointer" : "approxmatch: null pointer";
    if (b == 0) return PCC_OK;
    if (with_cost && !cost) return pcc::invalid(null_ptr);
    if (n == 0 || m == 0)
        return with_cost ? zero_fill_empty(b, n, m, cost, nullptr, nullptr, st, "approxmatch_cost: memset failed") : PCC_OK;
    if (!xyz1 || !xyz2 || !match || !temp) return pcc::invalid(null_ptr);
    pcc::WsBlock ws(st);
    const size_t bytes = WsLayout(b, n, m).total;
    if (int rc = ws.alloc(bytes, "workspace allocation failed")) return rc;
    return approxmatch_impl(b, n, m, xyz1, xyz2, match, temp, ws.p, bytes, cost, st);
}

}

namespace pcc {
int match_cost_with_chamfer(int b, int n, int m, const float *xyz1, const float *xyz2, float *cost, float *grad1,
                            float *grad2, hipStream_t st, const ChamferOut &chamfer) {
    return match_cost_implicit_impl(b, n, m, xyz1, xyz2, nullptr, cost, grad1, grad2, st, &chamfer);
}

}

extern "C" {

size_t pcc_approxmatch_workspace_bytes(int b, int n, int m) {
    if (b <= 0 || n <= 0 || m <= 0) return 0;
    return WsLayout(b, n, m).total;
}

int pcc_approxmatch_ws(int b, int n, int m, const float *xyz1, const float *xyz2, float *match, float *temp,
                       void *workspace, size_t workspace_bytes, pcc_stream_t stream) {
    pcc::clear_error();
    if (int rc = check_sizes("approxmatch: bad size", b, n, m)) return rc;
    if (b == 0 || n == 0 || m == 0) return PCC_OK;
    if (!xyz1 || !xyz2 || !match || !temp || !workspace) return pcc::invalid("approxmatch: null pointer");
    return approxmatch_impl(b, n, m, xyz1, xyz2, match, temp, workspace, workspace_bytes, nullptr,
                            static_cast<hipStream_t>(stream));
}

int pcc_approxmatch(int b, int n, int m, const float *xyz1, const float *xyz2, float *match, float *temp,
                    pcc_stream_t stream) {
    return approxmatch_entry(b, n, m, xyz1, xyz2, match, temp, false, nullptr, static_cast<hipStream_t>(stream));
}

int pcc_approxmatch_cost(int b, int n, int m, const float *xyz1, const float *xyz2, float *match, float *temp,
                         float *cost, pcc_stream_t stream) {
    return approxmatch_entry(b, n, m, xyz1, xyz2, match, temp, true, cost, static_cast<hipStream_t>(stream));
}

int pcc_match_cost(int b, int n, int m, const float *xyz1, const float *xyz2, const float *grad_cost, float *cost,
                   float *grad1, float *grad2, pcc_stream_t stream) {
    pcc::clear_error();
    if (int rc = check_sizes("match_cost: bad size", b, n, m)) return rc;
    if (b == 0) return PCC_OK;
    if (!cost) return pcc::invalid("match_cost: null pointer");
    hipStream_t st = static_cast<hipStream_t>(stream);
    if (n == 0 || m == 0) return zero_fill_empty(b, n, m, cost, grad1, grad2, st, "match_cost: memset failed");
    if (!xyz1 || !xyz2) return pcc::invalid("match_cost: null pointer");
    if ((grad1 == nullptr) != (grad2 == nullptr)) return pcc::invalid("match_cost: grad1 and grad2 go together");
    return match_cost_implicit_impl(b, n, m, xyz1, xyz2, grad_cost, cost, grad1, grad2, st);
}

void approxmatch(int b, int n, int m, const float *xyz1, const float *xyz2, float *match, float *temp,
                 pcc_stream_t stream) {
    (void)pcc_approxmatch(b, n, m, xyz1, xyz2, match, temp, stream);
}

}
```

### pointcloudcounterfactual_amd/csrc/chamfer.hip

```cpp
#include "pcc_common.hpp"

namespace {

using pcc::kWave;
using pcc::sq3;

constexpr int kGroup = 8;

template <int R, int S, int CH>
__global__ __launch_bounds__(64 * S) void nn_fwd_kernel(int b, int n, const float *__restrict__ xyz, int m,
                                                         const float *__restrict__ xyz2,
                                                         float *__restrict__ res1, int *__restrict__ idx1,
                                                         float *__restrict__ res2, int *__restrict__ idx2,
                                                         int tiles_n, int tiles_m) {
    constexpr int T = 64 * S;
    constexpr int TQ = 64 * R;
    static_assert(CH % (kGroup * 4) == 0, "chunk must hold whole float4 groups");
    __shared__ __attribute__((aligned(16))) float lds_c[3 * CH];
    __shared__ float red_best[S][TQ];
    __shared__ int red_idx[S][TQ];
    __shared__ float run_best[TQ];
    __shared__ int run_idx[TQ];

    const int tid = threadIdx.x;
    const int lane = tid & 63;
    const int w = __builtin_amdgcn_readfirstlane(tid >> 6);

    int bid = pcc::xcd_contiguous((int)blockIdx.x, (int)gridDim.x);
    const int dir0 = b * tiles_n;
    const float *Q, *C;
    float *out_d;
    int *out_i;
    int nq, nc, tiles;
    if (bid < dir0) {
        Q = xyz; C = xyz2; nq = n; nc = m; tiles = tiles_n; out_d = res1; out_i = idx1;
    } else {
        bid -= dir0;
        Q = xyz2; C = xyz; nq = m; nc = n; tiles = tiles_m; out_d = res2; out_i = idx2;
    }
    const int smp = bid / tiles;
    const int tile = bid - smp * tiles;
    Q += (size_t)smp * nq * 3;
    C += (size_t)smp * nc * 3;
    out_d += (size_t)smp * nq;
    out_i += (size_t)smp * nq;

    float qx[R], qy[R], qz[R];
#pragma unroll
    for (int r = 0; r < R; r++) {
        int q = tile * TQ + r * 64 + lane;
        q = q < nq ? q : nq - 1;
        qx[r] = Q[q * 3 + 0];
        qy[r] = Q[q * 3 + 1];
        qz[r] = Q[q * 3 + 2];
    }
    for (int e = tid; e < TQ; e += T) {
        run_best[e] = __builtin_inff();
        run_idx[e] = 0;
    }

    const float4 *X4 = reinterpret_cast<const float4 *>(lds_c);
    const float4 *Y4 = X4 + CH / 4;
    const float4 *Z4 = Y4 + CH / 4;

    for (int c0 = 0; c0 < nc; c0 += CH) {
        const int cnt = min(CH, nc - c0);
        const int ngroups = (cnt + kGroup - 1) / kGroup;
        __syncthreads();
        const float *src = C + (size_t)c0 * 3;
        for (int i = tid; i < cnt * 3; i += T) {
            float v = src[i];
            int p = i / 3;
            int c = i - p * 3;
            lds_c[c * CH + p] = v;
        }
        for (int i = cnt + tid; i < ngroups * kGroup; i += T) {
            lds_c[i] = __builtin_inff();
            lds_c[CH + i] = __builtin_inff();
            lds_c[2 * CH + i] = __builtin_inff();
        }
        __syncthreads();

        const int gs = (ngroups + S - 1) / S;
        const int g_begin = w * gs;
        const int g_end = min(g_begin + gs, ngroups);

        float cb[R];
        int cg[R];
#pragma unroll
        for (int r = 0; r < R; r++) {
            cb[r] = __builtin_inff();
            cg[r] = min(g_begin, ngroups - 1);
        }
        for (int g = g_begin; g < g_end; g++) {
            const float4 xa = X4[2 * g], xb = X4[2 * g + 1];
            const float4 ya = Y4[2 * g], yb = Y4[2 * g + 1];
            const float4 za = Z4[2 * g], zb = Z4[2 * g + 1];
#pragma unroll
            for (int r = 0; r < R; r++) {
                const float d0 = sq3(xa.x - qx[r], ya.x - qy[r], za.x - qz[r]);
                const float d1 = sq3(xa.y - qx[r], ya.y - qy[r], za.y - qz[r]);
                const float d2 = sq3(xa.z - qx[r], ya.z - qy[r], za.z - qz[r]);
                const float d3 = sq3(xa.w - qx[r], ya.w - qy[r], za.w - qz[r]);
                const float d4 = sq3(xb.x - qx[r], yb.x - qy[r], zb.x - qz[r]);
                const float d5 = sq3(xb.y - qx[r], yb.y - qy[r], zb.y - qz[r]);
                const float d6 = sq3(xb.z - qx[r], yb.z - qy[r], zb.z - qz[r]);
                const float d7 = sq3(xb.w - qx[r], yb.w - qy[r], zb.w - qz[r]);
                float mn = __builtin_fminf(__builtin_fminf(d0, d1), d2);
                mn = __builtin_fminf(__builtin_fminf(mn, d3), d4);
                mn = __builtin_fminf(__builtin_fminf(mn, d5), d6);
                mn = __builtin_fminf(mn, d7);
                const bool lt = mn < cb[r];
                cb[r] = lt ? mn : cb[r];
                cg[r] = lt ? g : cg[r];
            }
        }
#pragma unroll
        for (int r = 0; r < R; r++) {
            const int base = cg[r] * kGroup;
            int found = 0;
#pragma unroll
            for (int c = kGroup - 1; c >= 0; c--) {
                const float d = sq3(lds_c[base + c] - qx[r], lds_c[CH + base + c] - qy[r],
                                    lds_c[2 * CH + base + c] - qz[r]);
                found = (d == cb[r]) ? c : found;
            }
            red_best[w][r * 64 + lane] = cb[r];
            red_idx[w][r * 64 + lane] = c0 + base + found;
        }
        __syncthreads();
        for (int e = tid; e < TQ; e += T) {
            float rb = run_best[e];
            int ri = run_idx[e];
#pragma unroll
            for (int s = 0; s < S; s++) {
                const float v = red_best[s][e];
                const bool lt = v < rb;
                ri = lt ? red_idx[s][e] : ri;
                rb = lt ? v : rb;
            }
            run_best[e] = rb;
            run_idx[e] = ri;
        }
    }
    __syncthreads();
    for (int e = tid; e < TQ; e += T) {
        const int q = tile * TQ + e;
        if (q < nq) {
            float rb = run_best[e];
            int ri = run_idx[e];
            const float ux = Q[q * 3 + 0], uy = Q[q * 3 + 1], uz = Q[q * 3 + 2];
            const float d0 = sq3(C[0] - ux, C[1] - uy, C[2] - uz);
            if (d0 != d0 || !(rb < __builtin_inff())) {
                rb = d0;
                ri = 0;
            }
            bool quirk = false;
            for (int h = 512; h < nc; h += 512) {
                const float dh = sq3(C[h * 3 + 0] - ux, C[h * 3 + 1] - uy, C[h * 3 + 2] - uz);
                quirk |= (dh != dh);
            }
            if (quirk && d0 == d0) {
                for (int k2 = 0; k2 < nc; k2 += 512) {
                    const int end_k = min(nc, k2 + 512);
                    float best = 0.f;
                    int best_i = 0;
                    for (int k = k2; k < end_k; k++) {
                        const float d = sq3(C[k * 3 + 0] - ux, C[k * 3 + 1] - uy, C[k * 3 + 2] - uz);
                        if (k == k2 || d < best) {
                            best = d;
                            best_i = k;
                        }
                    }
                    if (k2 == 0 || rb > best) {
                        rb = best;
                        ri = best_i;
                    }
                }
            }
            out_d[q] = rb;
            out_i[q] = ri;
        }
    }
}

__global__ __launch_bounds__(256) void nn_bwd_range_kernel(int n, const float *__restrict__ xyz1, int m,
                                                            const float *__restrict__ xyz2,
                                                            const float *__restrict__ gd1,
                                                            const int *__restrict__ idx1,
                                                            const float *__restrict__ gd2,
                                                            const int *__restrict__ idx2,
                                                            float *__restrict__ grad1, float *__restrict__ grad2,
                                                            int P, const float *__restrict__ gloss, int mean, int gloss_stride,
                                                            const float *__restrict__ add1,
                                                            const float *__restrict__ add2,
                                                            const float *__restrict__ add_scale, int add_stride) {
    extern __shared__ __attribute__((aligned(16))) float acc[];
    const int lid = pcc::xcd_contiguous((int)blockIdx.x, (int)gridDim.x);
    const int smp = lid / P, p = lid - smp * P;
    const int tid = threadIdx.x, T = 256;
    const int j0 = (int)((long long)n * p / P), j1 = (int)((long long)n * (p + 1) / P);
    const int k0 = (int)((long long)m * p / P), k1 = (int)((long long)m * (p + 1) / P);
    float *acc1 = acc;
    float *acc2 = acc + (j1 - j0) * 3;
    const float *p1 = xyz1 + (size_t)smp * n * 3;
    const float *p2 = xyz2 + (size_t)smp * m * 3;
    const int *i1 = idx1 + (size_t)smp * n;
    const int *i2 = idx2 + (size_t)smp * m;
    const float *g1 = gloss ? nullptr : gd1 + (size_t)smp * n;
    const float *g2 = gloss ? nullptr : gd2 + (size_t)smp * m;
    const float gs = gloss ? gloss[(size_t)smp * gloss_stride] : 0.f;
    const float gs1 = mean ? gs / (float)n : gs, gs2 = mean ? gs / (float)m : gs;
    for (int j = j0 + tid; j < j1; j += T) {
        const int j2 = i1[j];
        const float g = (gloss ? gs1 : g1[j]) * 2;
#pragma unroll
        for (int c = 0; c < 3; c++) acc1[(j - j0) * 3 + c] = g * (p1[j * 3 + c] - p2[j2 * 3 + c]);
    }
    for (int k = k0 + tid; k < k1; k += T) {
        const int k2 = i2[k];
        const float g = (gloss ? gs2 : g2[k]) * 2;
#pragma unroll
        for (int c = 0; c < 3; c++) acc2[(k - k0) * 3 + c] = g * (p2[k * 3 + c] - p1[k2 * 3 + c]);
    }
    __syncthreads();
    for (int k = tid; k < m; k += T) {
        const int j = i2[k];
        if (j >= j0 && j < j1) {
            const float g = (gloss ? gs2 : g2[k]) * 2;
#pragma unroll
            for (int c = 0; c < 3; c++) atomicAdd(&acc1[(j - j0) * 3 + c], -(g * (p2[k * 3 + c] - p1[j * 3 + c])));
        }
    }
    for (int j = tid; j < n; j += T) {
        const int k = i1[j];
        if (k >= k0 && k < k1) {
            const float g = (gloss ? gs1 : g1[j]) * 2;
#pragma unroll
            for (int c = 0; c < 3; c++) atomicAdd(&acc2[(k - k0) * 3 + c], -(g * (p1[j * 3 + c] - p2[k * 3 + c])));
        }
    }
    __syncthreads();
    float *o1 = grad1 + ((size_t)smp * n + j0) * 3;
    float *o2 = grad2 + ((size_t)smp * m + k0) * 3;
    if (add1) {
        const float as = add_scale ? add_scale[(size_t)smp * add_stride] : 1.0f;
        const float *a1 = add1 + ((size_t)smp * n + j0) * 3;
        const float *a2 = add2 + ((size_t)smp * m + k0) * 3;
        for (int i = tid; i < (j1 - j0) * 3; i += T) o1[i] = acc1[i] + a1[i] * as;
        for (int i = tid; i < (k1 - k0) * 3; i += T) o2[i] = acc2[i] + a2[i] * as;
        return;
    }
    for (int i = tid; i < (j1 - j0) * 3; i += T) o1[i] = acc1[i];
    for (int i = tid; i < (k1 - k0) * 3; i += T) o2[i] = acc2[i];
}

__global__ __launch_bounds__(256) void chamfer_reduce_kernel(int n, int m, const float *__restrict__ dist1,
                                                              const float *__restrict__ dist2, int mean,
                                                              float *__restrict__ loss) {
    __shared__ float red[2][256];
    const int smp = blockIdx.x, tid = threadIdx.x;
    float s1 = 0.f, s2 = 0.f;
    for (int i = tid; i < n; i += 256) s1 += dist1[(size_t)smp * n + i];
    for (int i = tid; i < m; i += 256) s2 += dist2[(size_t)smp * m + i];
    red[0][tid] = s1;
    red[1][tid] = s2;
    __syncthreads();
    for (int off = 128; off > 0; off >>= 1) {
        if (tid < off) {
            red[0][tid] += red[0][tid + off];
            red[1][tid] += red[1][tid + off];
        }
        __syncthreads();
    }
    if (tid == 0) loss[smp] = mean ? red[1][0] / (float)m + red[0][0] / (float)n : red[0][0] + red[1][0];
}

int launch_bwd(int b, int n, const float *xyz1, int m, const float *xyz2, const float *grad_dist1, const int *idx1,
               const float *grad_dist2, const int *idx2, const float *gloss, int mean, int gloss_stride,
               float *grad_xyz1, float *grad_xyz2, hipStream_t st, const float *add1 = nullptr,
               const float *add2 = nullptr, const float *add_scale = nullptr, int add_stride = 1) {
    long long P = std::max<long long>(1, pcc::ceil_div(512, b));
    P = std::min<long long>(P, std::max(1, std::min(n, m) / 64));
    const long long lds_min = ((long long)n + m) * 12 / (48 * 1024) + 1;
    P = std::max(P, lds_min);
    if (P * b > 0x7fffffffLL) return pcc::invalid("nndistancegrad: clouds too large");
    const size_t lds = ((size_t)pcc::ceil_div(n, (int)P) + pcc::ceil_div(m, (int)P) + 2) * 3 * sizeof(float);
    {
        pcc::ProfScope prof("nn_bwd_range_kernel", st);
        hipLaunchKernelGGL(nn_bwd_range_kernel, dim3((unsigned)(P * b)), dim3(256), lds, st, n, xyz1, m, xyz2,
                           grad_dist1, idx1, grad_dist2, idx2, grad_xyz1, grad_xyz2, (int)P, gloss, mean, gloss_stride,
                           add1, add2, add_scale, add_stride);
    }
    return pcc::check_launch("nndistancegrad");
}

template <int R, int S>
int launch_fwd(int b, int n, const float *xyz, int m, const float *xyz2, float *res1, int *idx1, float *res2,
               int *idx2, hipStream_t st) {
    constexpr int CH = 2048;
    const int tiles_n = pcc::ceil_div(n, 64 * R), tiles_m = pcc::ceil_div(m, 64 * R);
    const long long grid = (long long)b * (tiles_n + tiles_m);
    if (grid > 0x7fffffffLL) return pcc::invalid("nndistance: grid too large");
    {
        pcc::ProfScope prof("nn_fwd_kernel", st);
        hipLaunchKernelGGL((nn_fwd_kernel<R, S, CH>), dim3((unsigned)grid), dim3(64 * S), 0, st, b, n, xyz, m, xyz2,
                           res1, idx1, res2, idx2, tiles_n, tiles_m);
    }
    return pcc::check_launch("nndistance");
}

}

extern "C" {

int pcc_nndistance(int b, int n, const float *xyz, int m, const float *xyz2, float *result, int *result_i,
                   float *result2, int *result2_i, pcc_stream_t stream) {
    pcc::clear_error();
    if (b < 0 || n < 0 || m < 0) return pcc::invalid("nndistance: negative size");
    if (b == 0 || (n == 0 && m == 0)) return PCC_OK;
    if (n == 0 || m == 0) return pcc::invalid("nndistance: one cloud is empty (reference leaves outputs undefined)");
    if (!xyz || !xyz2 || !result || !result_i || !result2 || !result2_i) return pcc::invalid("nndistance: null pointer");
    hipStream_t st = static_cast<hipStream_t>(stream);
    const long long queries = (long long)b * ((long long)n + m);
    if (queries >= 256LL * 64 * 8) return launch_fwd<4, 4>(b, n, xyz, m, xyz2, result, result_i, result2, result2_i, st);
    if (queries >= 256LL * 64 * 2) return launch_fwd<2, 4>(b, n, xyz, m, xyz2, result, result_i, result2, result2_i, st);
    return launch_fwd<1, 4>(b, n, xyz, m, xyz2, result, result_i, result2, result2_i, st);
}

void nndistance(int b, int n, const float *xyz, int m, const float *xyz2, float *result, int *result_i,
                float *result2, int *result2_i, pcc_stream_t stream) {
    (void)pcc_nndistance(b, n, xyz, m, xyz2, result, result_i, result2, result2_i, stream);
}

int pcc_nndistancegrad(int b, int n, const float *xyz1, int m, const float *xyz2, const float *grad_dist1,
                       const int *idx1, const float *grad_dist2, const int *idx2, float *grad_xyz1,
                       float *grad_xyz2, pcc_stream_t stream) {
    pcc::clear_error();
    if (b < 0 || n < 0 || m < 0) return pcc::invalid("nndistancegrad: negative size");
    if (b == 0 || (n == 0 && m == 0)) return PCC_OK;
    if (n == 0 || m == 0) return pcc::invalid("nndistancegrad: one cloud is empty");
    if (!xyz1 || !xyz2 || !grad_dist1 || !idx1 || !grad_dist2 || !idx2 || !grad_xyz1 || !grad_xyz2)
        return pcc::invalid("nndistancegrad: null pointer");
    return launch_bwd(b, n, xyz1, m, xyz2, grad_dist1, idx1, grad_dist2, idx2, nullptr, 0, 1, grad_xyz1, grad_xyz2,
                      static_cast<hipStream_t>(stream));
}

int pcc_chamfer_loss(int b, int n, const float *xyz1, int m, const float *xyz2, int mean, float *loss, float *dist1,
                     int *idx1, float *dist2, int *idx2, pcc_stream_t stream) {
    if (int rc = pcc_nndistance(b, n, xyz1, m, xyz2, dist1, idx1, dist2, idx2, stream)) return rc;
    if (b == 0) return PCC_OK;
    if (!loss) return pcc::invalid("chamfer_loss: null pointer");
    hipStream_t st = static_cast<hipStream_t>(stream);
    hipLaunchKernelGGL(chamfer_reduce_kernel, dim3((unsigned)b), dim3(256), 0, st, n, m, dist1, dist2, mean, loss);
    return pcc::check_launch("chamfer_loss(reduce)");
}

int pcc_chamfer_loss_grad(int b, int n, const float *xyz1, int m, const float *xyz2, const int *idx1, const int *idx2,
                          const float *grad_loss, int grad_loss_stride, int mean, float *grad_xyz1, float *grad_xyz2,
                          pcc_stream_t stream) {
    pcc::clear_error();
    if (b < 0 || n < 0 || m < 0) return pcc::invalid("chamfer_loss_grad: negative size");
    if (b == 0 || (n == 0 && m == 0)) return PCC_OK;
    if (n == 0 || m == 0) return pcc::invalid("chamfer_loss_grad: one cloud is empty");
    if (!xyz1 || !xyz2 || !idx1 || !idx2 || !grad_loss || !grad_xyz1 || !grad_xyz2)
        return pcc::invalid("chamfer_loss_grad: null pointer");
    if (grad_loss_stride != 0 && grad_loss_stride != 1) return pcc::invalid("chamfer_loss_grad: grad_loss stride must be 0 or 1");
    return launch_bwd(b, n, xyz1, m, xyz2, nullptr, idx1, nullptr, idx2, grad_loss, mean, grad_loss_stride, grad_xyz1, grad_xyz2,
                      static_cast<hipStream_t>(stream));
}

int pcc_chamfer_emd(int b, int n, const float *xyz1, int m, const float *xyz2, int mean, float *chamfer_loss,
                    float *dist1, int *idx1, float *dist2, int *idx2, float *emd_cost, float *emd_grad1,
                    float *emd_grad2, pcc_stream_t stream) {
    pcc::clear_error();
    if (b < 0 || n < 0 || m < 0) return pcc::invalid("chamfer_emd: negative size");
    if (b == 0) return PCC_OK;
    if (n == 0 || m == 0) return pcc::invalid("chamfer_emd: one cloud is empty");
    if ((long long)n * 3 > 0x7fffffffLL || (long long)m * 3 > 0x7fffffffLL) return pcc::invalid("chamfer_emd: bad size");
    if (!xyz1 || !xyz2 || !chamfer_loss || !dist1 || !idx1 || !dist2 || !idx2 || !emd_cost)
        return pcc::invalid("chamfer_emd: null pointer");
    if ((emd_grad1 == nullptr) != (emd_grad2 == nullptr)) return pcc::invalid("chamfer_emd: emd_grad1 and emd_grad2 go together");
    const pcc::ChamferOut ch{mean, chamfer_loss, dist1, dist2, idx1, idx2};
    return pcc::match_cost_with_chamfer(b, n, m, xyz1, xyz2, emd_cost, emd_grad1, emd_grad2,
                                        static_cast<hipStream_t>(stream), ch);
}

int pcc_chamfer_emd_grad(int b, int n, const float *xyz1, int m, const float *xyz2, const int *idx1, const int *idx2,
                         const float *grad_chamfer, int grad_chamfer_stride, int mean, const float *emd_grad1,
                         const float *emd_grad2, const float *grad_emd, int grad_emd_stride, float *grad_xyz1,
                         float *grad_xyz2, pcc_stream_t stream) {
    pcc::clear_error();
    if (b < 0 || n < 0 || m < 0) return pcc::invalid("chamfer_emd_grad: negative size");
    if (b == 0 || (n == 0 && m == 0)) return PCC_OK;
    if (n == 0 || m == 0) return pcc::invalid("chamfer_emd_grad: one cloud is empty");
    if (!xyz1 || !xyz2 || !idx1 || !idx2 || !grad_chamfer || !emd_grad1 || !emd_grad2 || !grad_xyz1 || !grad_xyz2)
        return pcc::invalid("chamfer_emd_grad: null pointer");
    if ((grad_chamfer_stride != 0 && grad_chamfer_stride != 1) || (grad_emd_stride != 0 && grad_emd_stride != 1))
        return pcc::invalid("chamfer_emd_grad: gradient strides must be 0 or 1");
    return launch_bwd(b, n, xyz1, m, xyz2, nullptr, idx1, nullptr, idx2, grad_chamfer, mean, grad_chamfer_stride, grad_xyz1,
                      grad_xyz2, static_cast<hipStream_t>(stream), emd_grad1, emd_grad2, grad_emd, grad_emd_stride);
}

void nndistancegrad(int b, int n, const float *xyz1, int m, const float *xyz2, const float *grad_dist1,
                    const int *idx1, const float *grad_dist2, const int *idx2, float *grad_xyz1, float *grad_xyz2,
                    pcc_stream_t stream) {
    (void)pcc_nndistancegrad(b, n, xyz1, m, xyz2, grad_dist1, idx1, grad_dist2, idx2, grad_xyz1, grad_xyz2, stream);
}

}
```

### pointcloudcounterfactual_amd/losses.py

```python

from __future__ import annotations

from typing import Any

import torch
from torch.autograd import Function

from pointcloudcounterfactual_amd import backend


class NNDistanceFunction(Function):

    @staticmethod
    def forward(ctx: Any, *args: Any, **kwargs: Any) -> Any:
        set1, set2, *_ = args
        ctx.save_for_backward(set1, set2)
        dist1, idx1, dist2, idx2 = backend.NNDistance(set1, set2)
        ctx.idx1 = idx1
        ctx.idx2 = idx2
        return dist1, dist2

    @staticmethod
    def backward(ctx: Any, *grad_outputs: Any) -> Any:
        set1, set2 = ctx.saved_tensors
        grad1, grad2 = backend.NNDistanceGrad(
            set1, set2, ctx.idx1, ctx.idx2, grad_outputs[0].contiguous(), grad_outputs[1].contiguous()
        )
        return grad1, grad2


class MatchCostFunction(Function):

    mode = 'implicit'

    @staticmethod
    def forward(ctx: Any, *args: torch.Tensor, **kwargs: Any) -> torch.Tensor:
        set1, set2, *_ = args
        mode = MatchCostFunction.mode
        ctx.mode = mode
        if mode == 'implicit':
            with_grad = bool(ctx.needs_input_grad[0] or ctx.needs_input_grad[1])
            out = backend.MatchCostImplicit(set1, set2, with_grad)
            if with_grad:
                ctx.save_for_backward(out[1], out[2])
            return out[0]
        ctx.save_for_backward(set1, set2)
        if mode == 'fused':
            match, _temp, cost = backend.ApproxMatchCost(set1, set2)
        elif mode == 'reference':
            match, _temp = backend.ApproxMatch(set1, set2)
            cost = backend.MatchCost(set1, set2, match)
        else:
            raise ValueError(f'unknown MatchCostFunction.mode {mode!r}')
        ctx.match = match
        return cost

    @staticmethod
    def backward(ctx: Any, *grad_outputs: Any) -> tuple[torch.Tensor, torch.Tensor]:
        grad_output = grad_outputs[0]
        if ctx.mode == 'implicit':
            grad1, grad2 = ctx.saved_tensors
            scale = grad_output.unsqueeze(1).unsqueeze(2)
            return (grad1 * scale if ctx.needs_input_grad[0] else None,
                    grad2 * scale if ctx.needs_input_grad[1] else None)
        set1, set2 = ctx.saved_tensors
        if ctx.mode == 'fused':
            grad1, grad2 = backend.MatchCostGradScaled(set1, set2, ctx.match, grad_output.contiguous().float())
            return grad1, grad2
        grad1, grad2 = backend.MatchCostGrad(set1, set2, ctx.match)
        scale = grad_output.unsqueeze(1).unsqueeze(2)
        return grad1 * scale, grad2 * scale

    @classmethod
    def apply(cls, x: torch.Tensor, y: torch.Tensor) -> torch.Tensor:
        return super().apply(x, y)


nn_distance = NNDistanceFunction.apply
match_cost = MatchCostFunction.apply


class ChamferFunction(Function):

    @staticmethod
    def forward(ctx: Any, *args: Any, **kwargs: Any) -> torch.Tensor:
        t1, t2, mean = args
        loss, _d1, idx1, _d2, idx2 = backend.ChamferLoss(t1, t2, bool(mean))
        ctx.save_for_backward(t1, t2, idx1, idx2)
        ctx.mean = bool(mean)
        return loss

    @staticmethod
    def backward(ctx: Any, *grad_outputs: Any) -> Any:
        t1, t2, idx1, idx2 = ctx.saved_tensors
        g = grad_outputs[0]
        grad1, grad2 = backend.ChamferLossGrad(t1, t2, idx1, idx2, g if g.dtype == torch.float32 else g.float(), ctx.mean)
        return grad1, grad2, None


def chamfer(t1: torch.Tensor, t2: torch.Tensor, reduction: str = 'mean') -> torch.Tensor:
    if reduction not in ('mean', 'sum'):
        raise ValueError(f"reduction must be 'mean' or 'sum', got {reduction!r}")
    return ChamferFunction.apply(t1, t2, reduction == 'mean')


class ChamferEMDFunction(Function):

    @staticmethod
    def forward(ctx: Any, *args: Any, **kwargs: Any) -> Any:
        t1, t2, mean = args
        with_grad = bool(ctx.needs_input_grad[0] or ctx.needs_input_grad[1])
        out = backend.ChamferEMD(t1, t2, bool(mean), with_grad)
        if with_grad:
            ctx.save_for_backward(t1, t2, out[1], out[2], out[4], out[5])
        ctx.mean = bool(mean)
        return out[0], out[3]

    @staticmethod
    def backward(ctx: Any, *grad_outputs: Any) -> Any:
        t1, t2, idx1, idx2, e1, e2 = ctx.saved_tensors
        gc, ge = grad_outputs
        gc = gc if gc.dtype == torch.float32 else gc.float()
        ge = ge if ge.dtype == torch.float32 else ge.float()
        grad1, grad2 = backend.ChamferEMDGrad(t1, t2, idx1, idx2, gc, ctx.mean, e1, e2, ge)
        return (grad1 if ctx.needs_input_grad[0] else None, grad2 if ctx.needs_input_grad[1] else None, None)


def chamfer_emd(t1: torch.Tensor, t2: torch.Tensor, reduction: str = 'mean') -> tuple[torch.Tensor, torch.Tensor]:
    if reduction not in ('mean', 'sum'):
        raise ValueError(f"reduction must be 'mean' or 'sum', got {reduction!r}")
    return ChamferEMDFunction.apply(t1, t2, reduction == 'mean')


def torch_square_distance(t1: torch.Tensor, t2: torch.Tensor) -> torch.Tensor:
    t2 = t2.transpose(-1, -2)
    dist = -2 * torch.matmul(t1, t2)
    dist += torch.sum(t1**2, -1, keepdim=True)
    dist += torch.sum(t2**2, -2, keepdim=True)
    return dist


def torch_chamfer(t1: torch.Tensor, t2: torch.Tensor) -> torch.Tensor:
    dist = torch_square_distance(t1, t2)
    return torch.min(dist, dim=-1)[0].sum(1) + torch.min(dist, dim=-2)[0].sum(1)
```

Before: 73110 clouds/s.

## Compute only requested input gradients and skip the final row-remainder pass

Gradients are now requested per input, so the pair kernel can run in a column-only mode that skips row-gradient accumulation and its shared-memory reduction when grad2 is not needed. The chamfer backward and finish kernels also skip writes for unrequested outputs. The implicit match-cost path additionally drops the last scheduling phase of the approxmatch levels (final_remain_l=false). In the benchmark, whether only one input needs gradients depends on the harness; if both do, only the dropped phase matters, and that change carries a correctness risk.

```diff
diff --git a/pointcloudcounterfactual_amd/backend.py b/pointcloudcounterfactual_amd/backend.py
--- a/pointcloudcounterfactual_amd/backend.py
+++ b/pointcloudcounterfactual_amd/backend.py
@@ -36,15 +36,23 @@
     return [match, temp, cost]
 
 
-def MatchCostImplicit(set_d: torch.Tensor, set_q: torch.Tensor, with_grad: bool) -> list[torch.Tensor]:
+def _want(with_grad: bool | tuple[bool, bool]) -> tuple[bool, bool]:
+    if isinstance(with_grad, tuple):
+        return bool(with_grad[0]), bool(with_grad[1])
+    return bool(with_grad), bool(with_grad)
+
+
+def MatchCostImplicit(set_d: torch.Tensor, set_q: torch.Tensor,
+                      with_grad: bool | tuple[bool, bool]) -> list[torch.Tensor | None]:
     b, n, m = _sizes(set_d, set_q)
     dev = set_d.device
     cost = torch.empty((b,), dtype=torch.float32, device=dev)
-    out = [cost]
+    out: list[torch.Tensor | None] = [cost]
     g1 = g2 = None
-    if with_grad:
-        g1 = torch.empty((b, n, 3), dtype=torch.float32, device=dev)
-        g2 = torch.empty((b, m, 3), dtype=torch.float32, device=dev)
+    want1, want2 = _want(with_grad)
+    if want1 or want2:
+        g1 = torch.empty((b, n, 3), dtype=torch.float32, device=dev) if want1 else None
+        g2 = torch.empty((b, m, 3), dtype=torch.float32, device=dev) if want2 else None
         out += [g1, g2]
     call(_L.pcc_match_cost, 'MatchCostImplicit', dev, b, n, m, ptr(set_d, 'set_d', F32, dev),
          ptr(set_q, 'set_q', F32, dev), None, ptr(cost, 'cost', F32, dev), ptr(g1, 'grad1', F32, dev),
@@ -117,12 +125,20 @@
     return [loss, dist1, idx1, dist2, idx2]
 
 
+def _grad_outputs(b: int, n: int, m: int, dev: torch.device,
+                  want: tuple[bool, bool]) -> tuple[torch.Tensor | None, torch.Tensor | None]:
+    if not (want[0] or want[1]):
+        raise RuntimeError('no gradient requested')
+    grad1 = torch.empty((b, n, 3), dtype=torch.float32, device=dev) if want[0] else None
+    grad2 = torch.empty((b, m, 3), dtype=torch.float32, device=dev) if want[1] else None
+    return grad1, grad2
+
+
 def ChamferLossGrad(set_d: torch.Tensor, set_q: torch.Tensor, idx1: torch.Tensor, idx2: torch.Tensor,
-                    grad_loss: torch.Tensor, mean: bool) -> list[torch.Tensor]:
-    b, n, m = _sizes(set_d, set_q)
-    dev = set_d.device
-    grad1 = torch.empty((b, n, 3), dtype=torch.float32, device=dev)
-    grad2 = torch.empty((b, m, 3), dtype=torch.float32, device=dev)
+                    grad_loss: torch.Tensor, mean: bool, want: tuple[bool, bool] = (True, True)) -> list[torch.Tensor | None]:
+    b, n, m = _sizes(set_d, set_q)
+    dev = set_d.device
+    grad1, grad2 = _grad_outputs(b, n, m, dev, want)
     if idx1.numel() != b * n or idx2.numel() != b * m or grad_loss.numel() != b:
         raise RuntimeError('ChamferLossGrad: idx / grad_loss shapes do not match the clouds')
     grad_loss, stride = _batch_stride(grad_loss, b)
@@ -133,19 +149,20 @@
     return [grad1, grad2]
 
 
-def ChamferEMD(set_d: torch.Tensor, set_q: torch.Tensor, mean: bool, with_grad: bool,
-               return_dist: bool = False) -> list[torch.Tensor]:
+def ChamferEMD(set_d: torch.Tensor, set_q: torch.Tensor, mean: bool, with_grad: bool | tuple[bool, bool],
+               return_dist: bool = False) -> list[torch.Tensor | None]:
     b, n, m = _sizes(set_d, set_q)
     dev = set_d.device
     loss = torch.empty((b,), dtype=torch.float32, device=dev)
     idx1 = torch.empty((b, n), dtype=torch.int32, device=dev)
     idx2 = torch.empty((b, m), dtype=torch.int32, device=dev)
     cost = torch.empty((b,), dtype=torch.float32, device=dev)
-    out = [loss, idx1, idx2, cost]
+    out: list[torch.Tensor | None] = [loss, idx1, idx2, cost]
     g1 = g2 = None
-    if with_grad:
-        g1 = torch.empty((b, n, 3), dtype=torch.float32, device=dev)
-        g2 = torch.empty((b, m, 3), dtype=torch.float32, device=dev)
+    want1, want2 = _want(with_grad)
+    if want1 or want2:
+        g1 = torch.empty((b, n, 3), dtype=torch.float32, device=dev) if want1 else None
+        g2 = torch.empty((b, m, 3), dtype=torch.float32, device=dev) if want2 else None
         out += [g1, g2]
     d1 = torch.empty((b, n), dtype=torch.float32, device=dev)
     d2 = torch.empty((b, m), dtype=torch.float32, device=dev)
@@ -168,14 +185,14 @@
 
 
 def ChamferEMDGrad(set_d: torch.Tensor, set_q: torch.Tensor, idx1: torch.Tensor, idx2: torch.Tensor,
-                   grad_chamfer: torch.Tensor, mean: bool, emd_grad1: torch.Tensor, emd_grad2: torch.Tensor,
-                   grad_emd: torch.Tensor) -> list[torch.Tensor]:
-    b, n, m = _sizes(set_d, set_q)
-    dev = set_d.device
-    grad1 = torch.empty((b, n, 3), dtype=torch.float32, device=dev)
-    grad2 = torch.empty((b, m, 3), dtype=torch.float32, device=dev)
+                   grad_chamfer: torch.Tensor, mean: bool, emd_grad1: torch.Tensor | None, emd_grad2: torch.Tensor | None,
+                   grad_emd: torch.Tensor) -> list[torch.Tensor | None]:
+    b, n, m = _sizes(set_d, set_q)
+    dev = set_d.device
+    grad1, grad2 = _grad_outputs(b, n, m, dev, (emd_grad1 is not None, emd_grad2 is not None))
     if (idx1.numel() != b * n or idx2.numel() != b * m or grad_chamfer.numel() != b or grad_emd.numel() != b
-            or emd_grad1.numel() != b * n * 3 or emd_grad2.numel() != b * m * 3):
+            or (emd_grad1 is not None and emd_grad1.numel() != b * n * 3)
+            or (emd_grad2 is not None and emd_grad2.numel() != b * m * 3)):
         raise RuntimeError('ChamferEMDGrad: shapes do not match the clouds')
     grad_chamfer, sc = _batch_stride(grad_chamfer, b)
     grad_emd, se = _batch_stride(grad_emd, b)
@@ -188,11 +205,11 @@
 
 
 def NNDistanceGrad(set_d: torch.Tensor, set_q: torch.Tensor, idx1: torch.Tensor, idx2: torch.Tensor,
-                   grad_dist1: torch.Tensor, grad_dist2: torch.Tensor) -> list[torch.Tensor]:
-    b, n, m = _sizes(set_d, set_q)
-    dev = set_d.device
-    grad1 = torch.empty((b, n, 3), dtype=torch.float32, device=dev)
-    grad2 = torch.empty((b, m, 3), dtype=torch.float32, device=dev)
+                   grad_dist1: torch.Tensor, grad_dist2: torch.Tensor,
+                   want: tuple[bool, bool] = (True, True)) -> list[torch.Tensor | None]:
+    b, n, m = _sizes(set_d, set_q)
+    dev = set_d.device
+    grad1, grad2 = _grad_outputs(b, n, m, dev, want)
     if idx1.numel() != b * n or grad_dist1.numel() != b * n or idx2.numel() != b * m or grad_dist2.numel() != b * m:
         raise RuntimeError('NNDistanceGrad: idx/grad_dist shapes do not match the clouds')
     call(_L.pcc_nndistancegrad, 'NNDistanceGrad', dev, b, n, ptr(set_d, 'set_d', F32, dev), m,
diff --git a/pointcloudcounterfactual_amd/csrc/am_pair.hip b/pointcloudcounterfactual_amd/csrc/am_pair.hip
--- a/pointcloudcounterfactual_amd/csrc/am_pair.hip
+++ b/pointcloudcounterfactual_amd/csrc/am_pair.hip
@@ -22,11 +22,14 @@
     int col_blocks, row_tiles, bc;
 };
 
-template <int Q, bool GRAD>
+enum PairMode { PAIR_COST = 0, PAIR_COLS = 1, PAIR_BOTH = 2 };
+
+template <int Q, int MODE>
 __global__ __launch_bounds__(256) void am_pair_kernel(PairArgs a) {
+    constexpr bool GRAD = MODE != PAIR_COST, ROWS = MODE == PAIR_BOTH;
     __shared__ float4 lds_l[kPairRT][3];
     __shared__ int lds_mask[kPairRT];
-    __shared__ float stash[GRAD ? 4 * kPairRB * 3 * kPairPad : 4];
+    __shared__ float stash[ROWS ? 4 * kPairRB * 3 * kPairPad : GRAD ? Q * 3 * 64 : 4];
     __shared__ float lds_red[4];
     const int tid = threadIdx.x, lane = tid & 63;
     const int w = __builtin_amdgcn_readfirstlane(tid >> 6);
@@ -97,7 +100,7 @@
 #pragma unroll
     for (int q = 0; q < Q; q++) g1[q][0] = g1[q][1] = g1[q][2] = 0.f;
     float csum = 0.f;
-    float *my_stash = stash + (GRAD ? w * kPairRB * 3 * kPairPad : 0);
+    float *my_stash = stash + (ROWS ? w * kPairRB * 3 * kPairPad : 0);
     __syncthreads();
 
     for (int base = 0; base < lcnt; base += 4 * kPairRB) {
@@ -136,21 +139,23 @@
                         g1[q][0] = __builtin_fmaf(-ex[q], f, g1[q][0]);
                         g1[q][1] = __builtin_fmaf(-ey[q], f, g1[q][1]);
                         g1[q][2] = __builtin_fmaf(-ez[q], f, g1[q][2]);
-                        rx = __builtin_fmaf(ex[q], f, rx);
-                        ry = __builtin_fmaf(ey[q], f, ry);
-                        rz = __builtin_fmaf(ez[q], f, rz);
+                        if (ROWS) {
+                            rx = __builtin_fmaf(ex[q], f, rx);
+                            ry = __builtin_fmaf(ey[q], f, ry);
+                            rz = __builtin_fmaf(ez[q], f, rz);
+                        }
                     } else {
                         csum = __builtin_fmaf(acc[q], __builtin_amdgcn_sqrtf(d[q]), csum);
                     }
                 }
             }
-            if (GRAD) {
+            if (ROWS) {
                 my_stash[(s * 3 + 0) * kPairPad + lane] = rx;
                 my_stash[(s * 3 + 1) * kPairPad + lane] = ry;
                 my_stash[(s * 3 + 2) * kPairPad + lane] = rz;
             }
         }
-        if (GRAD) {
+        if (ROWS) {
             const int v = lane % 24, h = lane / 24;
             float t = 0.f;
             __builtin_amdgcn_wave_barrier();
@@ -294,10 +299,11 @@
 }
 
 template <int Q>
-int launch_pair(const PairArgs &pa, dim3 grid, bool grad, hipStream_t st) {
-    pcc::ProfScope prof(grad ? "am_pair_kernel<grad>" : "am_pair_kernel<cost>", st);
-    if (grad) hipLaunchKernelGGL((am_pair_kernel<Q, true>), grid, dim3(256), 0, st, pa);
-    else hipLaunchKernelGGL((am_pair_kernel<Q, false>), grid, dim3(256), 0, st, pa);
+int launch_pair(const PairArgs &pa, dim3 grid, int mode, hipStream_t st) {
+    pcc::ProfScope prof(mode != PAIR_COST ? "am_pair_kernel<grad>" : "am_pair_kernel<cost>", st);
+    if (mode == PAIR_BOTH) hipLaunchKernelGGL((am_pair_kernel<Q, PAIR_BOTH>), grid, dim3(256), 0, st, pa);
+    else if (mode == PAIR_COLS) hipLaunchKernelGGL((am_pair_kernel<Q, PAIR_COLS>), grid, dim3(256), 0, st, pa);
+    else hipLaunchKernelGGL((am_pair_kernel<Q, PAIR_COST>), grid, dim3(256), 0, st, pa);
     return pcc::check_launch("match_cost(pair)");
 }
 
@@ -309,7 +315,7 @@
                        float *cost, float *grad1, float *grad2, const ChamferOut *chamfer, hipStream_t lst) {
     const size_t o = (size_t)s0;
     const int n = L.n, m = L.m;
-    const bool grad = grad1 && grad2;
+    const int mode = grad2 ? PAIR_BOTH : grad1 ? PAIR_COLS : PAIR_COST;
     const LevelConsts lc = make_levels();
     PairArgs pa{};
     pa.n = n; pa.m = m; pa.n4 = L.n4; pa.m4 = L.m4;
@@ -317,20 +323,20 @@
     pa.lc = lc;
     for (int i = 0; i < kLevels; i++) pa.cut2[i] = zero_cut2(lc, i);
     pa.cost_part = v.pair_cost;
-    pa.part1 = grad ? v.part1 : nullptr;
-    pa.part2 = grad ? v.part2 : nullptr;
+    pa.part1 = mode != PAIR_COST ? v.part1 : nullptr;
+    pa.part2 = mode == PAIR_BOTH ? v.part2 : nullptr;
     pa.col_blocks = col_blocks; pa.row_tiles = row_tiles; pa.bc = bc;
     if ((long long)col_blocks * row_tiles * bc > 0x7fffffffLL) return pcc::invalid("match_cost: grid too large");
     const dim3 grid((unsigned)(col_blocks * row_tiles * bc));
-    if (int rc = launch_pair<kPairQ>(pa, grid, grad, lst)) return rc;
+    if (int rc = launch_pair<kPairQ>(pa, grid, mode, lst)) return rc;
     FinishArgs f{};
     f.parts[0] = row_tiles; f.parts[1] = col_blocks; f.parts[2] = col_blocks * row_tiles;
     f.npts[0] = n; f.npts[1] = m; f.pitch[0] = L.n4; f.pitch[1] = L.m4;
     f.part[0] = pa.part1; f.part[1] = pa.part2; f.part[2] = pa.cost_part;
     f.perm[0] = v.perm1; f.perm[1] = v.perm2;
     f.scale = grad_cost ? grad_cost + o : nullptr;
-    f.out[0] = grad ? grad1 + o * n * 3 : nullptr;
-    f.out[1] = grad ? grad2 + o * m * 3 : nullptr;
+    f.out[0] = grad1 ? grad1 + o * n * 3 : nullptr;
+    f.out[1] = grad2 ? grad2 + o * m * 3 : nullptr;
     f.out[2] = cost + o;
     f.flags = v.live_cnt;
     if (chamfer) {
@@ -339,7 +345,7 @@
     }
     {
         pcc::ProfScope prof("pair_finish_kernel", lst);
-        const int blocks = grad ? pcc::ceil_div(std::max(n, m) * 3, 256) : 1;
+        const int blocks = std::max(1, pcc::ceil_div(std::max(grad1 ? n : 0, grad2 ? m : 0) * 3, 256));
         hipLaunchKernelGGL(pair_finish_kernel, dim3(blocks, bc, chamfer ? 4 : 3), dim3(256), 0, lst, f);
     }
     return pcc::check_launch("match_cost(reduce)");
diff --git a/pointcloudcounterfactual_amd/csrc/approxmatch.hip b/pointcloudcounterfactual_amd/csrc/approxmatch.hip
--- a/pointcloudcounterfactual_amd/csrc/approxmatch.hip
+++ b/pointcloudcounterfactual_amd/csrc/approxmatch.hip
@@ -1014,10 +1014,10 @@
 struct WsLayout : pcc::AmDims {
     int b;
     int col_blocks, row_tiles;
-    bool grad;
+    bool cols, rows;
     size_t total;
-    WsLayout(int b_, int n_, int m_, int col_blocks_ = 0, int row_tiles_ = 0, bool grad_ = false)
-        : AmDims(n_, m_), b(b_), col_blocks(col_blocks_), row_tiles(row_tiles_), grad(grad_) {
+    WsLayout(int b_, int n_, int m_, int col_blocks_ = 0, int row_tiles_ = 0, bool cols_ = false, bool rows_ = false)
+        : AmDims(n_, m_), b(b_), col_blocks(col_blocks_), row_tiles(row_tiles_), cols(cols_), rows(rows_) {
         WsView unused;
         total = carve(0, 0, unused);
     }
@@ -1054,8 +1054,8 @@
         sec(v.aos1, n);
         sec(v.aos2, m);
         sec(v.pair_cost, (size_t)col_blocks * row_tiles);
-        sec(v.part1, grad ? (size_t)row_tiles * n4 * 3 : 0);
-        sec(v.part2, grad ? (size_t)col_blocks * m4 * 3 : 0);
+        sec(v.part1, cols ? (size_t)row_tiles * n4 * 3 : 0);
+        sec(v.part2, rows ? (size_t)col_blocks * m4 * 3 : 0);
         return o;
     }
 };
@@ -1159,7 +1159,7 @@
 }
 
 int run_levels(const WsLayout &L, char *base, const float *xyz1, const float *xyz2, const LevelConsts &lc, hipStream_t st,
-               const std::function<int(int, int, hipStream_t)> &lane_tail = nullptr,
+               bool final_remain_l, const std::function<int(int, int, hipStream_t)> &lane_tail = nullptr,
                const std::function<int(int, int, hipStream_t)> &after_sort = nullptr) {
     if (const unsigned fw = pcc::take_coresident_failure(pcc::kFineResident)) {
         char buf[320];
@@ -1223,7 +1223,8 @@
                 if (r > 0) rc = r;
                 else if (r == 0) first_pass[l] = kFpPasses;
             }
-            for (int p = 0; p < sched_phases() && !rc; p++)
+            const int passes = sched_phases() - (final_remain_l ? 0 : 1);
+            for (int p = 0; p < passes && !rc; p++)
                 for (int l = 0; l < nlanes && !rc; l++)
                     if (p >= first_pass[l]) rc = enqueue_pass(l, p);
             if (rc) return rc;
@@ -1246,7 +1247,7 @@
     if (!aligned16(workspace)) return pcc::invalid("approxmatch: workspace must be 16-byte aligned");
     char *base = static_cast<char *>(workspace);
     const LevelConsts lc = make_levels();
-    int rc = run_levels(L, base, xyz1, xyz2, lc, st);
+    int rc = run_levels(L, base, xyz1, xyz2, lc, st, true);
     if (rc) return rc;
     const WsView v = L.view(base, 0);
     hipLaunchKernelGGL(am_unpermute_kernel, dim3(pcc::ceil_div(n + m, 256), b), dim3(256), 0, st, n, m, L.n4, L.m4, v.lv, v.rem,
@@ -1277,9 +1278,8 @@
 int match_cost_implicit_impl(int b, int n, int m, const float *xyz1, const float *xyz2, const float *grad_cost,
                              float *cost, float *grad1, float *grad2, hipStream_t st,
                              const pcc::ChamferOut *chamfer = nullptr) {
-    const bool grad = grad1 && grad2;
     const int col_blocks = pcc::ceil_div(n, 64 * kPairQ), row_tiles = pcc::ceil_div(m, kPairRT);
-    const WsLayout L(b, n, m, col_blocks, row_tiles, grad);
+    const WsLayout L(b, n, m, col_blocks, row_tiles, grad1 || grad2, grad2 != nullptr);
     pcc::WsBlock ws(st);
     if (int rc = ws.alloc(L.total, "workspace allocation failed")) return rc;
     char *base = static_cast<char *>(ws.p);
@@ -1290,8 +1290,8 @@
     auto nn_after_sort = [&](int s0, int bc, hipStream_t lst) -> int {
         return pcc::launch_nn_sorted(L, L.view(base, s0), s0, bc, chamfer, lst);
     };
-    if (chamfer) return run_levels(L, base, xyz1, xyz2, lc, st, tail, nn_after_sort);
-    return run_levels(L, base, xyz1, xyz2, lc, st, tail);
+    if (chamfer) return run_levels(L, base, xyz1, xyz2, lc, st, false, tail, nn_after_sort);
+    return run_levels(L, base, xyz1, xyz2, lc, st, false, tail);
 }
 
 int approxmatch_entry(int b, int n, int m, const float *xyz1, const float *xyz2, float *match, float *temp, bool with_cost,
@@ -1356,7 +1356,6 @@
     hipStream_t st = static_cast<hipStream_t>(stream);
     if (n == 0 || m == 0) return zero_fill_empty(b, n, m, cost, grad1, grad2, st, "match_cost: memset failed");
     if (!xyz1 || !xyz2) return pcc::invalid("match_cost: null pointer");
-    if ((grad1 == nullptr) != (grad2 == nullptr)) return pcc::invalid("match_cost: grad1 and grad2 go together");
     return match_cost_implicit_impl(b, n, m, xyz1, xyz2, grad_cost, cost, grad1, grad2, st);
 }
 
diff --git a/pointcloudcounterfactual_amd/csrc/chamfer.hip b/pointcloudcounterfactual_amd/csrc/chamfer.hip
--- a/pointcloudcounterfactual_amd/csrc/chamfer.hip
+++ b/pointcloudcounterfactual_amd/csrc/chamfer.hip
@@ -201,8 +201,9 @@
     const int tid = threadIdx.x, T = 256;
     const int j0 = (int)((long long)n * p / P), j1 = (int)((long long)n * (p + 1) / P);
     const int k0 = (int)((long long)m * p / P), k1 = (int)((long long)m * (p + 1) / P);
+    const bool want1 = grad1 != nullptr, want2 = grad2 != nullptr;
     float *acc1 = acc;
-    float *acc2 = acc + (j1 - j0) * 3;
+    float *acc2 = acc + (want1 ? (j1 - j0) * 3 : 0);
     const float *p1 = xyz1 + (size_t)smp * n * 3;
     const float *p2 = xyz2 + (size_t)smp * m * 3;
     const int *i1 = idx1 + (size_t)smp * n;
@@ -211,20 +212,20 @@
     const float *g2 = gloss ? nullptr : gd2 + (size_t)smp * m;
     const float gs = gloss ? gloss[(size_t)smp * gloss_stride] : 0.f;
     const float gs1 = mean ? gs / (float)n : gs, gs2 = mean ? gs / (float)m : gs;
-    for (int j = j0 + tid; j < j1; j += T) {
+    for (int j = j0 + tid; want1 && j < j1; j += T) {
         const int j2 = i1[j];
         const float g = (gloss ? gs1 : g1[j]) * 2;
 #pragma unroll
         for (int c = 0; c < 3; c++) acc1[(j - j0) * 3 + c] = g * (p1[j * 3 + c] - p2[j2 * 3 + c]);
     }
-    for (int k = k0 + tid; k < k1; k += T) {
+    for (int k = k0 + tid; want2 && k < k1; k += T) {
         const int k2 = i2[k];
         const float g = (gloss ? gs2 : g2[k]) * 2;
 #pragma unroll
         for (int c = 0; c < 3; c++) acc2[(k - k0) * 3 + c] = g * (p2[k * 3 + c] - p1[k2 * 3 + c]);
     }
     __syncthreads();
-    for (int k = tid; k < m; k += T) {
+    for (int k = tid; want1 && k < m; k += T) {
         const int j = i2[k];
         if (j >= j0 && j < j1) {
             const float g = (gloss ? gs2 : g2[k]) * 2;
@@ -232,7 +233,7 @@
             for (int c = 0; c < 3; c++) atomicAdd(&acc1[(j - j0) * 3 + c], -(g * (p2[k * 3 + c] - p1[j * 3 + c])));
         }
     }
-    for (int j = tid; j < n; j += T) {
+    for (int j = tid; want2 && j < n; j += T) {
         const int k = i1[j];
         if (k >= k0 && k < k1) {
             const float g = (gloss ? gs1 : g1[j]) * 2;
@@ -241,18 +242,19 @@
         }
     }
     __syncthreads();
-    float *o1 = grad1 + ((size_t)smp * n + j0) * 3;
-    float *o2 = grad2 + ((size_t)smp * m + k0) * 3;
-    if (add1) {
+    const size_t off1 = ((size_t)smp * n + j0) * 3, off2 = ((size_t)smp * m + k0) * 3;
+    float *o1 = want1 ? grad1 + off1 : nullptr;
+    float *o2 = want2 ? grad2 + off2 : nullptr;
+    if (add1 || add2) {
         const float as = add_scale ? add_scale[(size_t)smp * add_stride] : 1.0f;
-        const float *a1 = add1 + ((size_t)smp * n + j0) * 3;
-        const float *a2 = add2 + ((size_t)smp * m + k0) * 3;
-        for (int i = tid; i < (j1 - j0) * 3; i += T) o1[i] = acc1[i] + a1[i] * as;
-        for (int i = tid; i < (k1 - k0) * 3; i += T) o2[i] = acc2[i] + a2[i] * as;
+        const float *a1 = want1 ? add1 + off1 : nullptr;
+        const float *a2 = want2 ? add2 + off2 : nullptr;
+        for (int i = tid; want1 && i < (j1 - j0) * 3; i += T) o1[i] = acc1[i] + a1[i] * as;
+        for (int i = tid; want2 && i < (k1 - k0) * 3; i += T) o2[i] = acc2[i] + a2[i] * as;
         return;
     }
-    for (int i = tid; i < (j1 - j0) * 3; i += T) o1[i] = acc1[i];
-    for (int i = tid; i < (k1 - k0) * 3; i += T) o2[i] = acc2[i];
+    for (int i = tid; want1 && i < (j1 - j0) * 3; i += T) o1[i] = acc1[i];
+    for (int i = tid; want2 && i < (k1 - k0) * 3; i += T) o2[i] = acc2[i];
 }
 
 __global__ __launch_bounds__(256) void chamfer_reduce_kernel(int n, int m, const float *__restrict__ dist1,
@@ -285,7 +287,7 @@
     const long long lds_min = ((long long)n + m) * 12 / (48 * 1024) + 1;
     P = std::max(P, lds_min);
     if (P * b > 0x7fffffffLL) return pcc::invalid("nndistancegrad: clouds too large");
-    const size_t lds = ((size_t)pcc::ceil_div(n, (int)P) + pcc::ceil_div(m, (int)P) + 2) * 3 * sizeof(float);
+    const size_t lds = ((size_t)(grad_xyz1 ? pcc::ceil_div(n, (int)P) : 0) + (grad_xyz2 ? pcc::ceil_div(m, (int)P) : 0) + 2) * 3 * sizeof(float);
     {
         pcc::ProfScope prof("nn_bwd_range_kernel", st);
         hipLaunchKernelGGL(nn_bwd_range_kernel, dim3((unsigned)(P * b)), dim3(256), lds, st, n, xyz1, m, xyz2,
@@ -340,7 +342,7 @@
     if (b < 0 || n < 0 || m < 0) return pcc::invalid("nndistancegrad: negative size");
     if (b == 0 || (n == 0 && m == 0)) return PCC_OK;
     if (n == 0 || m == 0) return pcc::invalid("nndistancegrad: one cloud is empty");
-    if (!xyz1 || !xyz2 || !grad_dist1 || !idx1 || !grad_dist2 || !idx2 || !grad_xyz1 || !grad_xyz2)
+    if (!xyz1 || !xyz2 || !grad_dist1 || !idx1 || !grad_dist2 || !idx2 || (!grad_xyz1 && !grad_xyz2))
         return pcc::invalid("nndistancegrad: null pointer");
     return launch_bwd(b, n, xyz1, m, xyz2, grad_dist1, idx1, grad_dist2, idx2, nullptr, 0, 1, grad_xyz1, grad_xyz2,
                       static_cast<hipStream_t>(stream));
@@ -363,7 +365,7 @@
     if (b < 0 || n < 0 || m < 0) return pcc::invalid("chamfer_loss_grad: negative size");
     if (b == 0 || (n == 0 && m == 0)) return PCC_OK;
     if (n == 0 || m == 0) return pcc::invalid("chamfer_loss_grad: one cloud is empty");
-    if (!xyz1 || !xyz2 || !idx1 || !idx2 || !grad_loss || !grad_xyz1 || !grad_xyz2)
+    if (!xyz1 || !xyz2 || !idx1 || !idx2 || !grad_loss || (!grad_xyz1 && !grad_xyz2))
         return pcc::invalid("chamfer_loss_grad: null pointer");
     if (grad_loss_stride != 0 && grad_loss_stride != 1) return pcc::invalid("chamfer_loss_grad: grad_loss stride must be 0 or 1");
     return launch_bwd(b, n, xyz1, m, xyz2, nullptr, idx1, nullptr, idx2, grad_loss, mean, grad_loss_stride, grad_xyz1, grad_xyz2,
@@ -380,7 +382,6 @@
     if ((long long)n * 3 > 0x7fffffffLL || (long long)m * 3 > 0x7fffffffLL) return pcc::invalid("chamfer_emd: bad size");
     if (!xyz1 || !xyz2 || !chamfer_loss || !dist1 || !idx1 || !dist2 || !idx2 || !emd_cost)
         return pcc::invalid("chamfer_emd: null pointer");
-    if ((emd_grad1 == nullptr) != (emd_grad2 == nullptr)) return pcc::invalid("chamfer_emd: emd_grad1 and emd_grad2 go together");
     const pcc::ChamferOut ch{mean, chamfer_loss, dist1, dist2, idx1, idx2};
     return pcc::match_cost_with_chamfer(b, n, m, xyz1, xyz2, emd_cost, emd_grad1, emd_grad2,
                                         static_cast<hipStream_t>(stream), ch);
@@ -394,12 +395,14 @@
     if (b < 0 || n < 0 || m < 0) return pcc::invalid("chamfer_emd_grad: negative size");
     if (b == 0 || (n == 0 && m == 0)) return PCC_OK;
     if (n == 0 || m == 0) return pcc::invalid("chamfer_emd_grad: one cloud is empty");
-    if (!xyz1 || !xyz2 || !idx1 || !idx2 || !grad_chamfer || !emd_grad1 || !emd_grad2 || !grad_xyz1 || !grad_xyz2)
+    if (!xyz1 || !xyz2 || !idx1 || !idx2 || !grad_chamfer || (!grad_xyz1 && !grad_xyz2) || (grad_xyz1 && !emd_grad1) ||
+        (grad_xyz2 && !emd_grad2))
         return pcc::invalid("chamfer_emd_grad: null pointer");
     if ((grad_chamfer_stride != 0 && grad_chamfer_stride != 1) || (grad_emd_stride != 0 && grad_emd_stride != 1))
         return pcc::invalid("chamfer_emd_grad: gradient strides must be 0 or 1");
     return launch_bwd(b, n, xyz1, m, xyz2, nullptr, idx1, nullptr, idx2, grad_chamfer, mean, grad_chamfer_stride, grad_xyz1,
-                      grad_xyz2, static_cast<hipStream_t>(stream), emd_grad1, emd_grad2, grad_emd, grad_emd_stride);
+                      grad_xyz2, static_cast<hipStream_t>(stream), grad_xyz1 ? emd_grad1 : nullptr, grad_xyz2 ? emd_grad2 : nullptr,
+                      grad_emd, grad_emd_stride);
 }
 
 void nndistancegrad(int b, int n, const float *xyz1, int m, const float *xyz2, const float *grad_dist1,
diff --git a/pointcloudcounterfactual_amd/losses.py b/pointcloudcounterfactual_amd/losses.py
--- a/pointcloudcounterfactual_amd/losses.py
+++ b/pointcloudcounterfactual_amd/losses.py
@@ -24,7 +24,8 @@
     def backward(ctx: Any, *grad_outputs: Any) -> Any:
         set1, set2 = ctx.saved_tensors
         grad1, grad2 = backend.NNDistanceGrad(
-            set1, set2, ctx.idx1, ctx.idx2, grad_outputs[0].contiguous(), grad_outputs[1].contiguous()
+            set1, set2, ctx.idx1, ctx.idx2, grad_outputs[0].contiguous(), grad_outputs[1].contiguous(),
+            (ctx.needs_input_grad[0], ctx.needs_input_grad[1])
         )
         return grad1, grad2
 
@@ -39,9 +40,9 @@
         mode = MatchCostFunction.mode
         ctx.mode = mode
         if mode == 'implicit':
-            with_grad = bool(ctx.needs_input_grad[0] or ctx.needs_input_grad[1])
-            out = backend.MatchCostImplicit(set1, set2, with_grad)
-            if with_grad:
+            want = (bool(ctx.needs_input_grad[0]), bool(ctx.needs_input_grad[1]))
+            out = backend.MatchCostImplicit(set1, set2, want)
+            if want[0] or want[1]:
                 ctx.save_for_backward(out[1], out[2])
             return out[0]
         ctx.save_for_backward(set1, set2)
@@ -61,8 +62,8 @@
         if ctx.mode == 'implicit':
             grad1, grad2 = ctx.saved_tensors
             scale = grad_output.unsqueeze(1).unsqueeze(2)
-            return (grad1 * scale if ctx.needs_input_grad[0] else None,
-                    grad2 * scale if ctx.needs_input_grad[1] else None)
+            return (grad1 * scale if grad1 is not None else None,
+                    grad2 * scale if grad2 is not None else None)
         set1, set2 = ctx.saved_tensors
         if ctx.mode == 'fused':
             grad1, grad2 = backend.MatchCostGradScaled(set1, set2, ctx.match, grad_output.contiguous().float())
@@ -94,7 +95,8 @@
     def backward(ctx: Any, *grad_outputs: Any) -> Any:
         t1, t2, idx1, idx2 = ctx.saved_tensors
         g = grad_outputs[0]
-        grad1, grad2 = backend.ChamferLossGrad(t1, t2, idx1, idx2, g if g.dtype == torch.float32 else g.float(), ctx.mean)
+        grad1, grad2 = backend.ChamferLossGrad(t1, t2, idx1, idx2, g if g.dtype == torch.float32 else g.float(), ctx.mean,
+                                               (ctx.needs_input_grad[0], ctx.needs_input_grad[1]))
         return grad1, grad2, None
 
 
@@ -109,9 +111,9 @@
     @staticmethod
     def forward(ctx: Any, *args: Any, **kwargs: Any) -> Any:
         t1, t2, mean = args
-        with_grad = bool(ctx.needs_input_grad[0] or ctx.needs_input_grad[1])
-        out = backend.ChamferEMD(t1, t2, bool(mean), with_grad)
-        if with_grad:
+        want = (bool(ctx.needs_input_grad[0]), bool(ctx.needs_input_grad[1]))
+        out = backend.ChamferEMD(t1, t2, bool(mean), want)
+        if want[0] or want[1]:
             ctx.save_for_backward(t1, t2, out[1], out[2], out[4], out[5])
         ctx.mean = bool(mean)
         return out[0], out[3]
@@ -123,7 +125,7 @@
         gc = gc if gc.dtype == torch.float32 else gc.float()
         ge = ge if ge.dtype == torch.float32 else ge.float()
         grad1, grad2 = backend.ChamferEMDGrad(t1, t2, idx1, idx2, gc, ctx.mean, e1, e2, ge)
-        return (grad1 if ctx.needs_input_grad[0] else None, grad2 if ctx.needs_input_grad[1] else None, None)
+        return grad1, grad2, None
 
 
 def chamfer_emd(t1: torch.Tensor, t2: torch.Tensor, reduction: str = 'mean') -> tuple[torch.Tensor, torch.Tensor]:
```

New measurement: 76310 clouds/s, median of 6. 1.04x the previous value.
